# ChainSafe/halo2-verifier

Hardware: AMD Instinct MI355X
Metric: proofs verified/sec (BN254, k=14) (higher is better)
Workload: dtype u32 limbs (254-bit prime-field integers)

## Files before the change

### halo2_verifier_amd/csrc/curve.hip.h

```cpp
#pragma once
#include "bn254.hip.h"

namespace h2v {

static constexpr uint8_t G1_FLAG_IDENTITY = 0x80;
static constexpr uint8_t G1_FLAG_SIGN = 0x40;

struct G1A {
    Fq x, y;
    H2V_HD bool is_identity() const { return x.is_zero() && y.is_zero(); }
    H2V_HD static G1A identity() { G1A p; p.x = Fq::zero(); p.y = Fq::zero(); return p; }
    H2V_HD bool on_curve() const {
        if (is_identity()) return true;
        Fq three = Fq::from_u32(3);
        return y.sqr() == x.sqr() * x + three;
    }
};

struct G1J {
    Fq X, Y, Z;
    H2V_HD static G1J identity() { G1J p; p.X = Fq::zero(); p.Y = Fq::one(); p.Z = Fq::zero(); return p; }
    H2V_HD bool is_identity() const { return Z.is_zero(); }
    H2V_HD static G1J from_affine(const G1A& a) {
        if (a.is_identity()) return identity();
        G1J p; p.X = a.x; p.Y = a.y; p.Z = Fq::one(); return p;
    }
    H2V_HD G1J neg() const { G1J r = *this; r.Y = Y.neg(); return r; }
};

H2V_FN G1J g1_dbl(const G1J& p);
#define H2V_M(a, b) Fq::mul_inl((a), (b))
#define H2V_S(a) (a).sqr_inl()
__host__ __device__ __forceinline__ Fq g1_minus_eight() {
    const Fq k = {{0x1d9096cdu, 0x022be75eu, 0x12c66350u, 0x1e1f47a4u, 0x0b760e9fu, 0x1e7fbbcfu, 0x134a4383u, 0x01be3557u, 0x0022eb3au}};
    return k;
}
__host__ __device__ __forceinline__ G1J g1_dbl_inl(const G1J& p) {
    if (p.is_identity()) return p;
    const Fq A = H2V_S(p.X), B = H2V_S(p.Y), XB = H2V_M(p.X, B), C = H2V_S(B);
    const Fq E = Fq::lazy_add2(A, A), F = H2V_S(E), D = Fq::lazy_dbl(Fq::lazy_dbl(XB));
    int64_t acc[9];
#pragma unroll
    for (int l = 0; l < 9; ++l) acc[l] = (int64_t)F.v[l] + (int64_t)Fq::KP29(9, l) - 2 * (int64_t)D.v[l];
    G1J r;
    r.X = Fq::from_wide(acc);
    r.Y = Fq::dot2_inl(E, Fq::lazy_sub(D, r.X), C, g1_minus_eight());
    r.Z = H2V_M(Fq::lazy_dbl(p.Y), p.Z);
    return r;
}

__host__ __device__ __forceinline__ bool g1_madd_fast(G1J& acc, const G1A& q) {
    if (q.is_identity()) return true;
    if (acc.is_identity()) { acc.X = q.x; acc.Y = q.y; acc.Z = Fq::one(); return true; }
    const Fq Z1Z1 = H2V_S(acc.Z);
    const Fq U2 = H2V_M(q.x, Z1Z1), S2 = H2V_M(H2V_M(q.y, acc.Z), Z1Z1);
    const Fq H = Fq::lazy_sub(U2, acc.X), H2 = Fq::lazy_dbl(H), I = H2V_S(H2);
    if (I.is_zero()) return false;
    const Fq B = Fq::lazy_neg2(acc.Y), rr = Fq::lazy_add2(B, S2);
    const Fq X3 = Fq::dot2_inl(rr, rr, I, Fq::template lazy_lin<8, 1, 2>(H, acc.X));
    const Fq W = Fq::dot2_inl(rr, acc.X, H, B);
    acc.Y = Fq::dot2_inl(I, W, rr, Fq::lazy_neg(X3));
    acc.Z = H2V_M(acc.Z, H2);
    acc.X = X3;
    return true;
}
__host__ __device__ __forceinline__ bool g1_add_fast(G1J& acc, const G1J& q) {
    if (q.is_identity()) return true;
    if (acc.is_identity()) { acc.X = q.X; acc.Y = q.Y; acc.Z = q.Z; return true; }
    const Fq Z1Z1 = H2V_S(acc.Z), Z2Z2 = H2V_S(q.Z);
    const Fq U1 = H2V_M(acc.X, Z2Z2), U2 = H2V_M(q.X, Z1Z1);
    const Fq H = Fq::lazy_sub(U2, U1), H2 = Fq::lazy_dbl(H), I = H2V_S(H2);
    if (I.is_zero()) return false;
    const Fq S1 = H2V_M(H2V_M(acc.Y, q.Z), Z2Z2), S2 = H2V_M(H2V_M(q.Y, acc.Z), Z1Z1);
    const Fq B = Fq::lazy_neg2(S1), rr = Fq::lazy_add2(B, S2);
    const Fq X3 = Fq::dot2_inl(rr, rr, I, Fq::template lazy_lin<8, 1, 2>(H, U1));
    const Fq W = Fq::dot2_inl(rr, U1, H, B);
    acc.Y = Fq::dot2_inl(I, W, rr, Fq::lazy_neg(X3));
    acc.Z = H2V_M(H2V_M(acc.Z, q.Z), H2);
    acc.X = X3;
    return true;
}
__host__ __device__ __forceinline__ G1J g1_add_inl(const G1J& p, const G1J& q) {
    G1J r = p;
    if (g1_add_fast(r, q)) return r;
    const Fq Z1Z1 = H2V_S(p.Z), Z2Z2 = H2V_S(q.Z);
    const Fq S1 = H2V_M(H2V_M(p.Y, q.Z), Z2Z2), S2 = H2V_M(H2V_M(q.Y, p.Z), Z1Z1);
    if (S1 == S2) return g1_dbl(r);
    return G1J::identity();
}

__host__ __device__ __forceinline__ G1J g1_add_affine_inl(const G1J& p, const G1A& q) {
    G1J r = p;
    if (g1_madd_fast(r, q)) return r;
    const Fq Z1Z1 = H2V_S(p.Z);
    const Fq S2 = H2V_M(H2V_M(q.y, p.Z), Z1Z1);
    if (p.Y == S2) return g1_dbl(r);
    return G1J::identity();
}

H2V_FN G1J g1_dbl(const G1J& p) { return g1_dbl_inl(p); }
__host__ __device__ __forceinline__ Fq g1_beta_times(const Fq& x) {
    const Fq beta = {{0x18ccb791u, 0x175b1c3au, 0x0b83d6e2u, 0x0e8ed071u, 0x1282bee2u, 0x04220e84u, 0x1fe4017fu, 0x15084d4au, 0x00169119u}};
    return Fq::mul_inl(x, beta);
}
__host__ __device__ __forceinline__ G1A g1_phi(const G1A& p) { G1A r; r.x = g1_beta_times(p.x); r.y = p.y; return r; }
H2V_FN G1J g1_add(const G1J& p, const G1J& q) { return g1_add_inl(p, q); }
H2V_FN G1J g1_add_affine(const G1J& p, const G1A& q) { return g1_add_affine_inl(p, q); }

H2V_FN G1A g1_to_affine(const G1J& p) {
    if (p.is_identity()) return G1A::identity();
    Fq zi = p.Z.inv(), zi2 = zi.sqr();
    G1A a; a.x = p.X * zi2; a.y = p.Y * zi2 * zi;
    return a;
}

struct FqSqrtSchedule { uint8_t op[400]; int n; };
template <int W> constexpr FqSqrtSchedule fq_sqrt_schedule() {
    constexpr uint32_t e[8] = {0xb61f3f52u, 0x4f082305u, 0x5a1c72a3u, 0x65e05aa4u, 0xa0605617u, 0x6e14116du, 0xb84c680au, 0x0c19139cu};
    FqSqrtSchedule s{};
    s.n = 0;
    int i = 255;
    while (i >= 0 && !((e[i >> 5] >> (i & 31)) & 1)) --i;
    while (i >= 0) {
        if (!((e[i >> 5] >> (i & 31)) & 1)) { s.op[s.n++] = 0; --i; continue; }
        int l = i - (W - 1) < 0 ? 0 : i - (W - 1);
        while (!((e[l >> 5] >> (l & 31)) & 1)) ++l;
        uint32_t v = 0;
        for (int k = i; k >= l; --k) { v = (v << 1) | ((e[k >> 5] >> (k & 31)) & 1); s.op[s.n++] = 0; }
        s.op[s.n++] = (uint8_t)((v + 1) / 2);
        i = l - 1;
    }
    return s;
}
template <int W> __host__ __device__ inline __attribute__((noinline)) Fq fq_sqrt_candidate_w(const Fq& a) {
    constexpr FqSqrtSchedule S = fq_sqrt_schedule<W>();
    constexpr int T = 1 << (W - 1);
    Fq t[T];
    t[0] = a;
    const Fq a2 = a.sqr();
#pragma unroll
    for (int k = 1; k < T; ++k) t[k] = t[k - 1] * a2;
    Fq r = Fq::one();
    bool started = false;
#pragma unroll
    for (int k = 0; k < S.n; ++k) {
        if (S.op[k] == 0) { if (started) r = r.sqr(); }
        else { r = started ? r * t[S.op[k] - 1] : t[S.op[k] - 1]; started = true; }
    }
    return r;
}
H2V_FN Fq fq_sqrt_candidate(const Fq& a) { return fq_sqrt_candidate_w<4>(a); }

struct FqSqrtRuns { uint8_t nsq[160]; uint8_t idx[160]; int n; int first; };
template <int W> constexpr FqSqrtRuns fq_sqrt_runs() {
    constexpr FqSqrtSchedule S = fq_sqrt_schedule<W>();
    FqSqrtRuns r{};
    r.n = 0; r.first = -1;
    int pending = 0;
    for (int k = 0; k < S.n; ++k) {
        if (S.op[k] == 0) { if (r.first >= 0) ++pending; continue; }
        if (r.first < 0) { r.first = S.op[k] - 1; continue; }
        r.nsq[r.n] = (uint8_t)pending; r.idx[r.n] = (uint8_t)(S.op[k] - 1); ++r.n; pending = 0;
    }
    if (pending) { r.nsq[r.n] = (uint8_t)pending; r.idx[r.n] = 255; ++r.n; }
    return r;
}
#if defined(__HIPCC__)
__device__ __constant__ const FqSqrtRuns fq_sqrt_runs_w3 = fq_sqrt_runs<3>();
__device__ __forceinline__ Fq fq_sqrt_candidate_loop_w3(const Fq& a) {
    Fq t0 = a;
    const Fq a2 = a.sqr_inl();
    const Fq t1 = Fq::mul_inl(t0, a2), t2 = Fq::mul_inl(t1, a2), t3 = Fq::mul_inl(t2, a2);
    auto pick = [&](uint32_t i) -> Fq {
        Fq s;
#pragma unroll
        for (int l = 0; l < H2V_LIMBS; ++l) s.v[l] = i == 0 ? t0.v[l] : (i == 1 ? t1.v[l] : (i == 2 ? t2.v[l] : t3.v[l]));
        return s;
    };
    Fq r = pick((uint32_t)fq_sqrt_runs_w3.first);
    const int n = fq_sqrt_runs_w3.n;
#pragma unroll 1
    for (int k = 0; k < n; ++k) {
        const uint32_t nsq = fq_sqrt_runs_w3.nsq[k], idx = fq_sqrt_runs_w3.idx[k];
#pragma unroll 1
        for (uint32_t i = 0; i < nsq; ++i) r = r.sqr_inl();
        if (idx == 0u) r = Fq::mul_inl(r, t0);
        else if (idx == 1u) r = Fq::mul_inl(r, t1);
        else if (idx == 2u) r = Fq::mul_inl(r, t2);
        else if (idx == 3u) r = Fq::mul_inl(r, t3);
    }
    return r;
}
#endif

H2V_FN bool g1_decompress(const uint8_t in[32], G1A& out) {
    uint8_t tmp[32];
    for (int i = 0; i < 32; ++i) tmp[i] = in[i];
    bool is_inf = tmp[31] & G1_FLAG_IDENTITY, sign = tmp[31] & G1_FLAG_SIGN;
    tmp[31] &= 0x3f;
    Fq x;
    if (!Fq::from_bytes(tmp, x)) return false;
    if (is_inf) {
        if (!x.is_zero() || sign) return false;
        out = G1A::identity();
        return true;
    }
    Fq rhs = x.sqr() * x + Fq::from_u32(3);
    Fq y = fq_sqrt_candidate(rhs);
    if (y.sqr() != rhs) return false;
    if (y.is_odd() != sign) y = y.neg();
    out.x = x; out.y = y;
    return true;
}

template <int S> __device__ __forceinline__ Fq quad_bcast(const Fq& v) {
    Fq r;
#pragma unroll
    for (int l = 0; l < H2V_LIMBS; ++l) r.v[l] = (uint32_t)__builtin_amdgcn_mov_dpp((int)v.v[l], S * 0x55, 0xf, 0xf, true);
    return r;
}
__device__ __forceinline__ Fq fq_sel(bool c, const Fq& a, const Fq& b) {
    Fq r;
#pragma unroll
    for (int l = 0; l < H2V_LIMBS; ++l) r.v[l] = c ? a.v[l] : b.v[l];
    return r;
}
__device__ __forceinline__ void g1_dbl_quad(G1J& p, uint32_t r) {
    const Fq Y2 = Fq::lazy_dbl(p.Y);
    const Fq p1 = Fq::mul_inl(fq_sel(r == 0, p.X, fq_sel(r == 1, p.Y, Y2)), fq_sel(r == 0, p.X, fq_sel(r == 1, p.Y, p.Z)));
    const Fq A = quad_bcast<0>(p1), B = quad_bcast<1>(p1), Z3 = quad_bcast<2>(p1);
    const Fq E = Fq::lazy_add2(A, A);
    const Fq p2 = Fq::mul_inl(fq_sel(r == 0, B, fq_sel(r == 1, p.X, E)), fq_sel(r == 2, E, B));
    const Fq C = quad_bcast<0>(p2), XB = quad_bcast<1>(p2), F = quad_bcast<2>(p2);
    const Fq D = Fq::lazy_dbl(Fq::lazy_dbl(XB));
    int64_t acc[9];
#pragma unroll
    for (int l = 0; l < 9; ++l) acc[l] = (int64_t)F.v[l] + (int64_t)Fq::KP29(9, l) - 2 * (int64_t)D.v[l];
    p.X = Fq::from_wide(acc);
    p.Y = Fq::dot2_inl(E, Fq::lazy_sub(D, p.X), C, g1_minus_eight());
    p.Z = Z3;
}
template <class Slot> __device__ __forceinline__ G1J msm_horner_quad(const Slot* __restrict__ src, uint32_t items, uint32_t dbl, uint32_t r) {
    G1J acc = src[items - 1].p;
    for (int w = (int)items - 2; w >= 0; --w) {
        const G1J cur = src[w].p;
#pragma unroll 1
        for (uint32_t i = 0; i < dbl; ++i) g1_dbl_quad(acc, r);
        acc = g1_add_inl(acc, cur);
    }
    return acc;
}

}
```

### halo2_verifier_amd/csrc/internal.h

```cpp
#pragma once
#include <hip/hip_runtime.h>
#include <stdint.h>
#include <string>
#include <vector>
#include "../../include/h2v.h"
#include "curve.hip.h"

namespace h2v {

void set_last_error(const std::string& s);
#define H2V_HIP_CHECK(expr)                                                                     \
    do {                                                                                        \
        hipError_t e_ = (expr);                                                                 \
        if (e_ != hipSuccess) {                                                                 \
            ::h2v::set_last_error(std::string(#expr) + ": " + hipGetErrorString(e_));           \
            return H2V_ERR_DEVICE;                                                              \
        }                                                                                       \
    } while (0)

template <class T> struct DevBuf {
    T* p = nullptr;
    size_t cap = 0;
    DevBuf() {}
    DevBuf(const DevBuf&) = delete;
    DevBuf& operator=(const DevBuf&) = delete;
    DevBuf(DevBuf&& o) noexcept : p(o.p), cap(o.cap) { o.p = nullptr; o.cap = 0; }
    DevBuf& operator=(DevBuf&& o) noexcept { if (this != &o) { reset(); p = o.p; cap = o.cap; o.p = nullptr; o.cap = 0; } return *this; }
    ~DevBuf() { reset(); }
    int alloc(size_t count) {
        reset();
        H2V_HIP_CHECK(hipMalloc(&p, (count ? count : 1) * sizeof(T)));
        cap = count ? count : 1;
        return 0;
    }
    int reserve(size_t count) { return p && count <= cap ? 0 : alloc(count); }
    void reset() { if (p) hipFree(p); p = nullptr; cap = 0; }
};

struct MappedHostBuf {
    uint8_t* p = nullptr;
    void* dev = nullptr;
    size_t cap = 0;
    MappedHostBuf() {}
    MappedHostBuf(const MappedHostBuf&) = delete;
    MappedHostBuf& operator=(const MappedHostBuf&) = delete;
    ~MappedHostBuf() { reset(); }
    int reserve(size_t bytes) {
        if (p && bytes <= cap) return 0;
        reset();
        H2V_HIP_CHECK(hipHostMalloc((void**)&p, bytes ? bytes : 1, hipHostMallocMapped));
        H2V_HIP_CHECK(hipHostGetDevicePointer(&dev, p, 0));
        cap = bytes ? bytes : 1;
        return 0;
    }
    void reset() { if (p) hipHostFree(p); p = nullptr; dev = nullptr; cap = 0; }
};


struct MsmPlan {
    uint32_t n;
    uint32_t c;
    uint32_t windows;
    uint32_t buckets;
};
MsmPlan msm_plan(uint32_t n, bool latency = false);

struct MsmProblem {
    const uint32_t* scalars; const G1A* bases; G1J* out;
    uint32_t sstride, bstride, n;
    uint32_t n1;
    const uint32_t* scalars2; const G1A* bases2;
    const G1A* phi = nullptr; const G1A* phi2 = nullptr;
    uint32_t glv_off = 0;
    uint32_t sub_first = 0, sub_count = 0;
    uint32_t nnz = 0;
    MsmProblem() : scalars(nullptr), bases(nullptr), out(nullptr), sstride(8), bstride(1), n(0), n1(0), scalars2(nullptr), bases2(nullptr) {}
    MsmProblem(const uint32_t* s, const G1A* b, G1J* o, uint32_t ss, uint32_t bs, uint32_t n_) : scalars(s), bases(b), out(o), sstride(ss), bstride(bs), n(n_), n1(n_), scalars2(nullptr), bases2(nullptr) {}
    MsmProblem(const uint32_t* s, const G1A* b, G1J* o, uint32_t ss, uint32_t bs, uint32_t n1_, const uint32_t* s2, const G1A* b2, uint32_t n2)
        : scalars(s), bases(b), out(o), sstride(ss), bstride(bs), n(n1_ + n2), n1(n1_), scalars2(s2), bases2(b2) {}
};
#define MSM_MAX_PROBLEMS 1024
#define MSM_PROBLEM_CHUNK 44
struct MsmProblemChunk { MsmProblem p[MSM_PROBLEM_CHUNK]; };
static_assert(sizeof(MsmProblemChunk) <= 4000, "a chunk of problem descriptors travels as one kernel argument (4 KB limit)");
struct MsmProblems { std::vector<MsmProblem> p; };

struct alignas(128) G1JSlot {
    G1J p;
    uint32_t pad[5];
    __host__ __device__ G1JSlot& operator=(const G1J& v) { p = v; for (int i = 0; i < 5; ++i) pad[i] = 0; return *this; }
    __host__ __device__ operator const G1J&() const { return p; }
};

#define MSM_MAX_PARTS 6
struct MsmSplit {
    uint32_t want_parts = 0;
    uint32_t parts = 0, shift = 0, count = 0;
    const G1JSlot* pts = nullptr;
    const G1JSlot* ready = nullptr;
};

struct AccRecord { uint32_t failed, parts, shift, reserved; G1J left[H2V_ACC_RECORD_PIECES], right[H2V_ACC_RECORD_PIECES]; };
static_assert(sizeof(AccRecord) == H2V_ACC_RECORD_BYTES && H2V_ACC_RECORD_BYTES == 16 + 2 * H2V_ACC_RECORD_PIECES * 108, "accumulator record layout");
static_assert(H2V_ACC_RECORD_PIECES >= MSM_MAX_PARTS, "a record holds every piece a launch can leave");

struct MsmWorkspace {
    uint32_t cap_terms = 0, cap_parents = 0, cap_per_problem = 0;
    uint32_t cap_problems = 0;
    size_t cap_buckets = 0, cap_list = 0;
    DevBuf<uint32_t> counts;
    DevBuf<uint32_t> offsets;
    DevBuf<uint32_t> cursor;
    DevBuf<uint32_t> list;
    DevBuf<G1JSlot> bucket_pts;
    DevBuf<G1JSlot> window_sums;
    DevBuf<G1JSlot> pieces;
    std::vector<MsmProblem> resident;
    int resident_no_split = 0;
    DevBuf<MsmProblem> problems;
    DevBuf<MsmProblem> parents;
    DevBuf<G1JSlot> merged_sums;
    const MsmProblem* final_problems = nullptr;
    DevBuf<uint32_t> block_sums;
    DevBuf<G1JSlot> partial;
    DevBuf<uint32_t> redo;
    DevBuf<uint32_t> glv;
    DevBuf<G1A> phi_pts;
    DevBuf<uint32_t> seg_total;
    DevBuf<uint32_t> seg_start;
    h2v_tuning tune = {};
    bool profile = false, profile_recorded = false;
    hipEvent_t ev_acc[2] = {nullptr, nullptr};
    int reserve(uint32_t max_total_terms, uint32_t max_problems, uint32_t max_terms_per_problem = 0);
    bool covers(uint32_t max_total_terms, uint32_t max_problems, uint32_t max_terms_per_problem = 0) const;
    MsmWorkspace() {}
    MsmWorkspace(const MsmWorkspace&) = delete;
    MsmWorkspace& operator=(const MsmWorkspace&) = delete;
    ~MsmWorkspace() { for (hipEvent_t e : ev_acc) if (e) hipEventDestroy(e); }
};
int msm_enqueue_multi(hipStream_t s, MsmWorkspace& ws, const MsmProblems& pr, MsmSplit* split = nullptr);
int msm_combine_enqueue(hipStream_t s, MsmWorkspace& ws, const MsmSplit& sp, size_t lds_reserve = 0);
#define H2V_AUX_LDS_RESERVE ((size_t)110 * 1024)
int msm_enqueue(hipStream_t s, MsmWorkspace& ws, const uint32_t* d_scalars, const G1A* d_bases, uint32_t n, G1J* d_out);
int accumulator_scale_enqueue(hipStream_t s, const G1J* d_points, const uint32_t* d_scalar_words, void* d_record);
int accumulator_scale_many_enqueue(hipStream_t s, const G1J* d_pairs, const uint32_t* d_slots, const uint32_t* d_scalar_words, uint32_t n, void* d_records);

int bases_from_bytes_enqueue(hipStream_t s, const uint8_t* d_bytes, G1A* d_out, uint32_t* d_flags, uint32_t n);
int scalars_from_bytes_enqueue(hipStream_t s, const uint8_t* d_bytes, uint32_t* d_out, uint32_t* d_flags, uint32_t n);
int copy_words_enqueue(hipStream_t s, const void* d_src, void* d_dst, size_t n_words, size_t lds_reserve = 0);
int point_to_bytes_enqueue(hipStream_t s, const G1J* d_in, uint8_t* d_out_xy64, uint32_t* d_is_identity, uint32_t n, size_t lds_reserve = 0);
int export_records_enqueue(hipStream_t s, const G1J* d_acc, const G1JSlot* d_pieces, uint32_t parts, uint32_t shift, const int* d_status, uint32_t n, uint32_t groups, void* d_out);
int fold_records_enqueue(hipStream_t s, const void* d_recs, uint32_t n_recs, uint32_t groups, uint32_t parts, uint32_t shift, G1J* d_acc, G1JSlot* d_pieces, G1JSlot* d_ready,
                         uint32_t* d_fold_failed);

}
```

### halo2_verifier_amd/csrc/msm.hip

```cpp
#include "../../include/h2v.h"
#include <hip/hip_ext.h>
#include "batch.h"

namespace h2v {

#define MSM_LDS_SORT_MAX_TERMS 16384u
#define MSM_SORT_THREADS 512u
#define MSM_CHUNK_MIN 16u
#define MSM_CHUNK_MAX 64u
#define MSM_ACC_LANES_PER_ROUND 196608u
#define MSM_CHUNK_SMALL 4u
#define MSM_SHORT_LIST 98304u
__host__ __device__ __forceinline__ uint32_t msm_chunk_len(uint32_t E, uint32_t R) {
    if (E <= MSM_SHORT_LIST) return MSM_CHUNK_SMALL;
    if (E <= R * MSM_CHUNK_MIN) return MSM_CHUNK_MIN;
    const uint32_t k = (uint32_t)(((uint64_t)E + (uint64_t)R * MSM_CHUNK_MAX - 1) / ((uint64_t)R * MSM_CHUNK_MAX));
    const uint32_t c = (uint32_t)(((uint64_t)E + (uint64_t)k * R - 1) / ((uint64_t)k * R));
    return c < MSM_CHUNK_MIN ? MSM_CHUNK_MIN : c;
}
static inline uint32_t msm_accumulate_blocks(size_t max_entries, size_t R) {
    size_t lanes;
    if (max_entries <= R * MSM_CHUNK_MIN)
        lanes = std::max<size_t>((max_entries + MSM_CHUNK_MIN - 1) / MSM_CHUNK_MIN, (std::min<size_t>(max_entries, MSM_SHORT_LIST) + MSM_CHUNK_SMALL - 1) / MSM_CHUNK_SMALL);
    else lanes = (max_entries + R * MSM_CHUNK_MAX - 1) / (R * MSM_CHUNK_MAX) * R;
    return (uint32_t)(((lanes + 63) / 64 + 1 + 7) / 8 * 8);
}
#define MSM_CONTROL_WORDS 8u
#define MSM_FIXUP_SERIAL 64u
#define MSM_FIXUP_TEAM 3u
#define MSM_FIXUP_TEAM_BLOCKS 256u
#define MSM_FIXUP_HEAVY_BLOCKS 256u
#define MSM_WIN_THREADS 256

static inline uint32_t msm_window_threads(uint32_t buckets, uint32_t n_workgroups = 0xffffffffu, int forced = 0) {
    if (buckets <= 64) return std::max(1u, buckets);
    if (n_workgroups != 0xffffffffu && (forced == 64 || forced == 128 || forced == 256)) return (uint32_t)forced;
    if (buckets > 2048 || (buckets >= 256 && n_workgroups <= 256)) return 256u;
    return 64u;
}

MsmPlan msm_plan(uint32_t n, bool latency) {
    MsmPlan best{n, 2, 65, 2};
    double best_cost = 1e300;
    for (uint32_t c = 2; c <= 15; ++c) {
        uint32_t w = (130 + c - 1) / c;
        uint32_t b = 1u << (c - 1);
        uint32_t T = msm_window_threads(b), slice = (b + T - 1) / T;
        double lg = 0; for (uint32_t t = T; t > 1; t >>= 1) lg += 1;
        double cost = latency ? 9.0 * w + 9.0 * (2.0 * slice + 1.5 * c + 1.0 + lg) + 5.0 * std::min<double>(32.0, 2.0 * n)
                              : (double)w * (11.0 * 2.0 * n + 16.0 * T * (2.0 * slice + 1.5 * c + 1.0 + lg));
        if (cost < best_cost) { best_cost = cost; best = MsmPlan{n, c, w, b}; }
    }
    return best;
}
static inline bool msm_latency_bound(size_t total_terms) { return total_terms <= 4096; }

static inline uint32_t msm_subproblems(uint32_t n) { return n > MSM_LDS_SORT_MAX_TERMS ? (n + MSM_LDS_SORT_MAX_TERMS - 1) / MSM_LDS_SORT_MAX_TERMS : 1u; }
bool MsmWorkspace::covers(uint32_t max_terms, uint32_t max_problems, uint32_t max_per_problem) const {
    if (!max_per_problem || max_per_problem > max_terms) max_per_problem = max_terms;
    return counts.p && max_terms <= cap_terms && max_problems <= cap_parents && max_per_problem <= cap_per_problem;
}
int MsmWorkspace::reserve(uint32_t max_terms, uint32_t max_problems, uint32_t max_per_problem) {
    if (!max_per_problem || max_per_problem > max_terms) max_per_problem = max_terms;
    if (covers(max_terms, max_problems, max_per_problem)) return 0;
    max_terms = std::max(max_terms, cap_terms); max_problems = std::max(max_problems, cap_parents); max_per_problem = std::max(max_per_problem, cap_per_problem);
    cap_terms = cap_parents = cap_per_problem = 0;
    resident.clear(); final_problems = nullptr; profile_recorded = false;
    const uint32_t subs = msm_subproblems(max_per_problem);
    cap_problems = (uint32_t)std::min<size_t>((size_t)max_problems * subs, MSM_MAX_PROBLEMS);
    if (cap_problems < max_problems) cap_problems = max_problems;
    const uint32_t per_sub = subs > 1 ? MSM_LDS_SORT_MAX_TERMS : max_per_problem;
    const uint32_t form_n[2] = {per_sub, max_per_problem}, form_q[2] = {cap_problems, max_problems};
    size_t mb = 0;
    cap_list = 0;
    for (int f = 0; f < 2; ++f) {
        size_t fb = 0;
        for (int lat = 0; lat < 2; ++lat) {
            for (uint32_t n = 1; n <= form_n[f]; n = n < 16 ? n + 1 : n + n / 8) { MsmPlan p = msm_plan(n, lat != 0); fb = std::max(fb, (size_t)p.windows * p.buckets); }
            MsmPlan p = msm_plan(form_n[f], lat != 0); fb = std::max(fb, (size_t)p.windows * p.buckets);
        }
        mb = std::max(mb, fb * form_q[f]);
        for (uint32_t n = 1;; n = n < 16 ? n + 1 : n + n / 8) {
            if (n > form_n[f]) n = form_n[f];
            size_t terms = n <= MSM_LDS_SORT_MAX_TERMS ? (size_t)n * form_q[f] : std::min<size_t>((size_t)max_terms, (size_t)n * form_q[f]);
            cap_list = std::max(cap_list, terms * 2 * std::max(msm_plan(n, false).windows, msm_plan(n, true).windows));
            if (n == form_n[f]) break;
        }
    }
    cap_buckets = mb;
    const size_t max_chunks = std::max<size_t>(cap_list / MSM_CHUNK_MIN + 1, std::min<size_t>(cap_list, MSM_SHORT_LIST) / MSM_CHUNK_SMALL + 1);
    int rc;
    if ((rc = counts.alloc(mb + MSM_CONTROL_WORDS)) || (rc = offsets.alloc(mb)) ||
        (rc = cursor.alloc(2 * mb)) ||
        (rc = list.alloc(cap_list)) || (rc = bucket_pts.alloc(mb)) || (rc = window_sums.alloc((size_t)128 * cap_problems)) ||
        (rc = merged_sums.alloc((size_t)128 * max_problems)) || (rc = pieces.alloc((size_t)2 * MSM_MAX_PARTS * cap_problems)) ||
        (rc = problems.alloc(cap_problems)) || (rc = parents.alloc(max_problems)) || (rc = block_sums.alloc(mb / 1024 + 2)) ||
        (rc = partial.alloc(max_chunks * 2)) || (rc = redo.alloc(max_chunks)) ||
        (rc = glv.alloc(cap_list / 2 + 1)) ||
        (rc = phi_pts.alloc((size_t)max_terms + 1)) || (rc = seg_total.alloc((size_t)128 * cap_problems + 2)) || (rc = seg_start.alloc((size_t)128 * cap_problems + 2))) {
        cap_problems = 0; cap_buckets = cap_list = 0;
        return rc;
    }
    for (int i = 0; i < 2; ++i) if (!ev_acc[i]) H2V_HIP_CHECK(hipEventCreate(&ev_acc[i]));
    cap_terms = max_terms; cap_parents = max_problems; cap_per_problem = max_per_problem;
    return 0;
}

__device__ __forceinline__ void mul_lo5(uint32_t out[5], const uint32_t* a, int na, const uint32_t* b, int nb) {
    uint64_t acc[5] = {0, 0, 0, 0, 0};
    for (int i = 0; i < na && i < 5; ++i) {
        uint64_t carry = 0;
        for (int j = 0; j < nb && i + j < 5; ++j) {
            uint64_t t = (uint64_t)a[i] * b[j] + (uint32_t)acc[i + j] + carry;
            acc[i + j] = (uint32_t)t; carry = t >> 32;
        }
    }
    for (int i = 0; i < 5; ++i) out[i] = (uint32_t)acc[i];
}
__device__ __forceinline__ void mul_hi256(uint32_t out[5], const uint32_t k[8], const uint32_t g[5]) {
    uint32_t t[13];
    for (int i = 0; i < 13; ++i) t[i] = 0;
    for (int i = 0; i < 8; ++i) {
        uint64_t carry = 0;
        for (int j = 0; j < 5; ++j) {
            uint64_t v = (uint64_t)k[i] * g[j] + t[i + j] + carry;
            t[i + j] = (uint32_t)v; carry = v >> 32;
        }
        t[i + 5] = (uint32_t)carry;
    }
    for (int i = 0; i < 5; ++i) out[i] = t[8 + i];
}
__device__ __forceinline__ void mul_lo8(uint32_t out[8], const uint32_t a[8], const uint32_t* b, int nb) {
    for (int i = 0; i < 8; ++i) out[i] = 0;
    for (int j = 0; j < nb; ++j) {
        uint64_t carry = 0;
        for (int i = 0; i + j < 8; ++i) {
            uint64_t t = (uint64_t)a[i] * b[j] + out[i + j] + carry;
            out[i + j] = (uint32_t)t; carry = t >> 32;
        }
    }
}
__device__ __forceinline__ bool glv_geq_r(const uint32_t v[8]) {
    const uint32_t RW[8] = {0xf0000001u, 0x43e1f593u, 0x79b97091u, 0x2833e848u, 0x8181585du, 0xb85045b6u, 0xe131a029u, 0x30644e72u};
    for (int i = 7; i >= 0; --i) { if (v[i] > RW[i]) return true; if (v[i] < RW[i]) return false; }
    return true;
}
struct GlvHalf { uint32_t mag[5]; bool neg; };
__device__ __forceinline__ void glv_finish(GlvHalf& h, uint32_t t[5]) {
    h.neg = (t[4] >> 31) != 0;
    if (h.neg) { uint64_t c = 1; for (int i = 0; i < 5; ++i) { uint64_t v = (uint64_t)(~t[i]) + c; t[i] = (uint32_t)v; c = v >> 32; } }
    for (int i = 0; i < 5; ++i) h.mag[i] = t[i];
}
__device__ __forceinline__ void glv_decompose(const uint32_t* __restrict__ k, GlvHalf& h1, GlvHalf& h2) {
    const uint32_t A1[5] = {0x7d4f1128u, 0x8211bbebu, 0xeeb859fcu, 0x6f4d8248u, 0u};
    const uint32_t B1N[5] = {0x94d213e3u, 0x89d32568u, 0u, 0u, 0u};
    const uint32_t B2[5] = {0x1221250bu, 0x0be4e154u, 0xeeb859fdu, 0x6f4d8248u, 0u};
    const uint32_t G1[5] = {0x00ff6565u, 0x5398fd03u, 0xa773d2d2u, 0x4ccef014u, 0x2u};
    const uint32_t G2[5] = {0xc7e0b3d7u, 0xd91d232eu, 0x2u, 0u, 0u};
    uint32_t kk[8];
    for (int i = 0; i < 8; ++i) kk[i] = k[i];
    uint32_t c1[5], c2[5], p1[5], p2[5], t1[8], t2[8];
    mul_hi256(c1, kk, G1);
    mul_hi256(c2, kk, G2);
    mul_lo5(p1, c1, 5, A1, 5); mul_lo5(p2, c2, 5, B1N, 5);
    {
        int64_t borrow = 0;
        for (int i = 0; i < 5; ++i) { int64_t v = (int64_t)kk[i] - p1[i] - p2[i] + borrow; t1[i] = (uint32_t)v; borrow = v >> 32; }
    }
    mul_lo5(p1, c1, 5, B1N, 5); mul_lo5(p2, c2, 5, B2, 5);
    {
        int64_t borrow = 0;
        for (int i = 0; i < 5; ++i) { int64_t v = (int64_t)p1[i] - p2[i] + borrow; t2[i] = (uint32_t)v; borrow = v >> 32; }
    }
    {
        const uint32_t s1 = (t1[4] >> 31) ? 0xffffffffu : 0u, s2 = (t2[4] >> 31) ? 0xffffffffu : 0u;
        for (int i = 5; i < 8; ++i) { t1[i] = s1; t2[i] = s2; }
        uint32_t u[8], v[8], w[8];
        mul_lo8(u, t1, B2, 4); mul_lo8(w, t2, B1N, 2);
        { int64_t borrow = 0; for (int i = 0; i < 8; ++i) { int64_t d = (int64_t)u[i] - w[i] + borrow; u[i] = (uint32_t)d; borrow = d >> 32; } }
        mul_lo8(v, t2, A1, 4); mul_lo8(w, t1, B1N, 2);
        { uint64_t carry = 0; for (int i = 0; i < 8; ++i) { uint64_t d = (uint64_t)v[i] + w[i] + carry; v[i] = (uint32_t)d; carry = d >> 32; } }
        const bool e1 = glv_geq_r(u), e2 = glv_geq_r(v);
        int64_t b1 = 0, b2 = 0;
        for (int i = 0; i < 5; ++i) {
            int64_t d = (int64_t)t1[i] - (e1 ? A1[i] : 0u) - (e2 ? B1N[i] : 0u) + b1; t1[i] = (uint32_t)d; b1 = d >> 32;
            d = (int64_t)t2[i] + (e1 ? B1N[i] : 0u) - (e2 ? B2[i] : 0u) + b2; t2[i] = (uint32_t)d; b2 = d >> 32;
        }
    }
    glv_finish(h1, t1);
    glv_finish(h2, t2);
}
__device__ __forceinline__ uint32_t raw_window(const uint32_t m[5], uint32_t w, uint32_t c) {
    uint32_t off = w * c, word = off >> 5, sh = off & 31;
    if (word >= 5) return 0;
    uint32_t v = m[word] >> sh;
    if (sh + c > 32 && word + 1 < 5) v |= m[word + 1] << (32 - sh);
    return v & ((1u << c) - 1);
}
#define ACC_SCALE_TABLE 8u
#define ACC_SCALE_DIGITS 33u
__global__ void __launch_bounds__(64) k_accumulator_scale(const G1J* __restrict__ in, const uint32_t* __restrict__ slots, const uint32_t* __restrict__ scalars,
                                                          AccRecord* __restrict__ out) {
    __shared__ G1J table[4][ACC_SCALE_TABLE];
    __shared__ G1J half_sum[4];
    const uint32_t item = blockIdx.x;
    in += 2 * (size_t)(slots ? slots[item] : item);
    const uint32_t* m_words = scalars + 8 * (size_t)item;
    out += item;
    const uint32_t lane = threadIdx.x, chain = (lane >> 2) & 3u, r = lane & 3u;
    const uint32_t side = chain >> 1, half = chain & 1u;
    const bool writer = lane < 16 && r == 0;
    uint32_t k[8];
    for (int i = 0; i < 8; ++i) k[i] = m_words[i];
    GlvHalf h1, h2;
    glv_decompose(k, h1, h2);
    const bool neg = half ? h2.neg : h1.neg;
    uint32_t mag[5];
    {
        uint64_t c = 0;
        for (int i = 0; i < 5; ++i) { const uint64_t v = (uint64_t)(half ? h2.mag[i] : h1.mag[i]) + (i < 4 ? 0x88888888u : 0x8u) + c; mag[i] = (uint32_t)v; c = v >> 32; }
    }
    G1J p = in[side];
    if (half) p.X = g1_beta_times(p.X);
    if (neg) p.Y = p.Y.neg();
    {
        G1J t = p;
        if (writer) table[chain][0] = t;
        t = g1_dbl(t);
        if (writer) table[chain][1] = t;
#pragma unroll 1
        for (uint32_t j = 2; j < ACC_SCALE_TABLE; ++j) { t = g1_add(t, p); if (writer) table[chain][j] = t; }
    }
    __syncthreads();
    G1J acc = G1J::identity();
#pragma unroll 1
    for (int w = (int)ACC_SCALE_DIGITS - 1; w >= 0; --w) {
        if (w != (int)ACC_SCALE_DIGITS - 1) {
#pragma unroll 1
            for (int i = 0; i < 4; ++i) g1_dbl_quad(acc, r);
        }
        const int d = (int)raw_window(mag, (uint32_t)w, 4) - 8;
        if (d != 0) {
            G1J t = table[chain][(d < 0 ? -d : d) - 1];
            if (d < 0) t.Y = t.Y.neg();
            acc = g1_add_inl(acc, t);
        }
    }
    if (writer) half_sum[chain] = acc;
    __syncthreads();
    if (lane < 2) {
        const G1J a = half_sum[2 * lane], b = half_sum[2 * lane + 1];
        G1J* dst = lane ? out->right : out->left;
        dst[0] = g1_add_inl(a, b);
        for (uint32_t j = 1; j < H2V_ACC_RECORD_PIECES; ++j) dst[j] = G1J::identity();
    }
    if (lane == 0) { out->failed = 0; out->parts = 1; out->shift = 0; out->reserved = 0; }
}
int accumulator_scale_enqueue(hipStream_t s, const G1J* d_points, const uint32_t* d_scalar_words, void* d_record) {
    return accumulator_scale_many_enqueue(s, d_points, nullptr, d_scalar_words, 1, d_record);
}
int accumulator_scale_many_enqueue(hipStream_t s, const G1J* d_pairs, const uint32_t* d_slots, const uint32_t* d_scalar_words, uint32_t n, void* d_records) {
    if (!n) return 0;
    hipLaunchKernelGGL(k_accumulator_scale, dim3(n), dim3(64), 0, s, d_pairs, d_slots, d_scalar_words, (AccRecord*)d_records);
    H2V_HIP_CHECK(hipGetLastError());
    return 0;
}

#define MSM_ENTRY_HALF 0x40000000u
#define MSM_ENTRY_NEG 0x80000000u
#define MSM_ENTRY_TERM 0x3fffffffu

#define MSM_TILE 1024u
#define MSM_TILE_THREADS 256u
#define MSM_LDS_WORDS 16384u

template <bool SCATTER>
__global__ void __launch_bounds__(MSM_TILE_THREADS) msm_count_or_scatter(const MsmProblem* __restrict__ prs, uint32_t n_problems, uint32_t tiles_per_problem, MsmPlan p, uint32_t windows_per_pass, uint32_t* __restrict__ counts,
                                                                         const uint32_t* __restrict__ offsets, uint32_t* __restrict__ cursor, uint32_t* __restrict__ list) {
    extern __shared__ uint32_t hist[];
    const uint32_t tiles = tiles_per_problem, per_xcd = (n_problems + 7) / 8;
    const uint32_t q = (blockIdx.x % 8) * per_xcd + (blockIdx.x / 8) / tiles, tile0 = ((blockIdx.x / 8) % tiles) * MSM_TILE, tid = threadIdx.x;
    if (q >= n_problems) return;
    const MsmProblem pq = prs[q];
    const uint32_t n = pq.n;
    if (tile0 >= n) return;
    const uint32_t nbq = p.windows * p.buckets;
    const uint32_t half_range = 1u << (p.c - 1);
    constexpr uint32_t PER = MSM_TILE / MSM_TILE_THREADS;
    for (uint32_t w0 = 0; w0 < p.windows; w0 += windows_per_pass) {
        const uint32_t w1 = min(p.windows, w0 + windows_per_pass), nwords = (w1 - w0) * p.buckets;
        for (uint32_t i = tid; i < nwords; i += MSM_TILE_THREADS) hist[i] = 0;
        __syncthreads();
        for (int phase = 0; phase < (SCATTER ? 2 : 1); ++phase) {
            for (uint32_t k = 0; k < PER; ++k) {
                const uint32_t t = tile0 + tid + k * MSM_TILE_THREADS;
                if (t >= n) break;
                const uint32_t* s = t < pq.n1 ? pq.scalars + (size_t)pq.sstride * t : pq.scalars2 + (size_t)pq.sstride * (t - pq.n1);
                uint32_t nz = 0;
                for (int i = 0; i < 8; ++i) nz |= s[i];
                if (!nz) continue;
                const uint32_t* bw = reinterpret_cast<const uint32_t*>(t < pq.n1 ? pq.bases + (size_t)pq.bstride * t : pq.bases2 + (size_t)pq.bstride * (t - pq.n1));
                uint32_t any = 0;
                for (int i = 0; i < (int)(sizeof(G1A) / 4); ++i) any |= bw[i];
                if (!any) continue;
                GlvHalf h[2];
                glv_decompose(s, h[0], h[1]);
                for (uint32_t hf = 0; hf < 2; ++hf) {
                    uint32_t carry = 0;
                    for (uint32_t w = 0; w < w1; ++w) {
                        uint32_t raw = raw_window(h[hf].mag, w, p.c) + carry;
                        bool neg_digit = raw > half_range;
                        uint32_t mag = neg_digit ? (1u << p.c) - raw : raw;
                        carry = neg_digit ? 1u : 0u;
                        if (!mag || w < w0) continue;
                        uint32_t local = (w - w0) * p.buckets + mag - 1;
                        if (!SCATTER || phase == 0) atomicAdd(&hist[local], 1u);
                        else {
                            uint32_t b = q * nbq + w * p.buckets + mag - 1;
                            uint32_t pos = atomicAdd(&hist[local], 1u);
                            list[offsets[b] + pos] = t | (hf ? MSM_ENTRY_HALF : 0u) | ((neg_digit != h[hf].neg) ? MSM_ENTRY_NEG : 0u);
                        }
                    }
                }
            }
            __syncthreads();
            if (phase == 0) {
                for (uint32_t i = tid; i < nwords; i += MSM_TILE_THREADS) {
                    uint32_t v = hist[i];
                    if (!v) continue;
                    uint32_t b = q * nbq + w0 * p.buckets + i;
                    if (SCATTER) hist[i] = atomicAdd(&cursor[b], v);
                    else atomicAdd(&counts[b], v);
                }
                __syncthreads();
            }
        }
    }
}

__global__ void __launch_bounds__(256) msm_glv_prep(const MsmProblem* __restrict__ prs, uint32_t n_problems, MsmPlan p, uint32_t* __restrict__ dig, G1A* __restrict__ phi_pts) {
    const uint32_t q = blockIdx.y, t = blockIdx.x * blockDim.x + threadIdx.x;
    if (q >= n_problems) return;
    const MsmProblem pq = prs[q];
    if (t >= pq.n) return;
    uint32_t* out = dig + (size_t)pq.glv_off * p.windows + t;
    const uint32_t* sc = t < pq.n1 ? pq.scalars + (size_t)pq.sstride * t : pq.scalars2 + (size_t)pq.sstride * (t - pq.n1);
    uint32_t nz = 0;
    for (int i = 0; i < 8; ++i) nz |= sc[i];
    if (nz) {
        const uint32_t* bw = reinterpret_cast<const uint32_t*>(t < pq.n1 ? pq.bases + (size_t)pq.bstride * t : pq.bases2 + (size_t)pq.bstride * (t - pq.n1));
        uint32_t any = 0;
        for (int i = 0; i < (int)(sizeof(G1A) / 4); ++i) any |= bw[i];
        nz = any;
        if (any && !(t < pq.n1 ? pq.phi : pq.phi2)) phi_pts[(size_t)pq.glv_off + t] = g1_phi(*reinterpret_cast<const G1A*>(bw));
    }
    if (!nz) { for (uint32_t w = 0; w < p.windows; ++w) out[(size_t)w * pq.n] = 0; return; }
    GlvHalf h[2];
    glv_decompose(sc, h[0], h[1]);
    const uint32_t half_range = 1u << (p.c - 1);
    uint32_t carry[2] = {0, 0};
    for (uint32_t w = 0; w < p.windows; ++w) {
        uint32_t word = 0;
#pragma unroll
        for (uint32_t hf = 0; hf < 2; ++hf) {
            const uint32_t raw = raw_window(h[hf].mag, w, p.c) + carry[hf];
            const bool neg_digit = raw > half_range;
            const uint32_t mag = neg_digit ? (1u << p.c) - raw : raw;
            carry[hf] = neg_digit ? 1u : 0u;
            const uint32_t d16 = mag ? (mag | ((neg_digit != h[hf].neg) ? 0x8000u : 0u)) : 0u;
            word |= d16 << (16 * hf);
        }
        out[(size_t)w * pq.n] = word;
    }
}
__global__ void __launch_bounds__(MSM_SORT_THREADS) msm_sort_lds(const MsmProblem* __restrict__ prs, const uint32_t* __restrict__ dig, MsmPlan p, uint32_t stride,
                                                                 uint32_t* __restrict__ counts, uint32_t* __restrict__ offsets, uint32_t* __restrict__ list,
                                                                 uint32_t* __restrict__ seg_total) {
    extern __shared__ uint32_t sort_lds[];
    uint32_t* hist = sort_lds;
    uint32_t* part = sort_lds + p.buckets;
    unsigned short* rec = reinterpret_cast<unsigned short*>(part + MSM_SORT_THREADS);
    const uint32_t w = blockIdx.x, q = blockIdx.y, tid = threadIdx.x;
    const MsmProblem pq = prs[q];
    const uint32_t n = pq.n, seg = q * p.windows + w;
    const uint32_t* dw = dig + (size_t)pq.glv_off * p.windows + (size_t)w * n;
    for (uint32_t i = tid; i < p.buckets; i += MSM_SORT_THREADS) hist[i] = 0;
    __syncthreads();
    for (int pass = 0; pass < 2; ++pass) {
        for (uint32_t t = tid; t < n; t += MSM_SORT_THREADS) {
            const uint32_t word = dw[t];
#pragma unroll
            for (uint32_t hf = 0; hf < 2; ++hf) {
                const uint32_t d16 = (word >> (16 * hf)) & 0xffffu, mag = d16 & 0x7fffu;
                if (!mag) continue;
                const uint32_t pos = atomicAdd(&hist[mag - 1], 1u);
                if (pass == 1) rec[pos] = (unsigned short)(t | (hf ? 0x4000u : 0u) | (d16 & 0x8000u));
            }
        }
        __syncthreads();
        if (pass == 0) {
            const uint32_t per = (p.buckets + MSM_SORT_THREADS - 1) / MSM_SORT_THREADS, b0 = tid * per;
            uint32_t local = 0;
            for (uint32_t i = 0; i < per; ++i) if (b0 + i < p.buckets) local += hist[b0 + i];
            part[tid] = local;
            __syncthreads();
            for (uint32_t d = 1; d < MSM_SORT_THREADS; d <<= 1) {
                const uint32_t v = tid >= d ? part[tid - d] : 0;
                __syncthreads();
                part[tid] += v;
                __syncthreads();
            }
            uint32_t run = part[tid] - local;
            const size_t bin0 = (size_t)seg * p.buckets;
            for (uint32_t i = 0; i < per; ++i) if (b0 + i < p.buckets) {
                const uint32_t cnt = hist[b0 + i];
                counts[bin0 + b0 + i] = cnt; offsets[bin0 + b0 + i] = run;
                hist[b0 + i] = run;
                run += cnt;
            }
            if (tid == MSM_SORT_THREADS - 1) seg_total[seg] = part[tid];
            __syncthreads();
        }
    }
    const uint32_t total = part[MSM_SORT_THREADS - 1];
    uint32_t* dst = list + (size_t)seg * stride;
    for (uint32_t i = tid; i < total; i += MSM_SORT_THREADS) {
        const uint32_t r = rec[i];
        dst[i] = (r & 0x3fffu) | ((r & 0x4000u) ? MSM_ENTRY_HALF : 0u) | ((r & 0x8000u) ? MSM_ENTRY_NEG : 0u);
    }
}
__global__ void __launch_bounds__(1024) msm_seg_scan(const uint32_t* __restrict__ seg_total, uint32_t nseg, uint32_t* __restrict__ seg_start, uint32_t* __restrict__ control) {
    __shared__ uint32_t part[1024];
    __shared__ uint32_t carry;
    const uint32_t t = threadIdx.x;
    if (t == 0) carry = 0;
    __syncthreads();
    for (uint32_t base = 0; base < nseg; base += 1024) {
        const uint32_t i = base + t, c = i < nseg ? seg_total[i] : 0;
        part[t] = c;
        __syncthreads();
        for (uint32_t d = 1; d < 1024; d <<= 1) {
            const uint32_t v = t >= d ? part[t - d] : 0;
            __syncthreads();
            part[t] += v;
            __syncthreads();
        }
        if (i < nseg) seg_start[i] = carry + part[t] - c;
        __syncthreads();
        if (t == 1023) carry += part[1023];
        __syncthreads();
    }
    if (t == 0) { seg_start[nseg] = carry; control[0] = 0; control[1] = carry; control[2] = 0; control[3] = 0; control[4] = 0; }
}

__device__ __forceinline__ G1A msm_entry_load(const MsmProblem& q, uint32_t e, const G1A* __restrict__ phi_pts) {
    const uint32_t t = e & MSM_ENTRY_TERM;
    const bool first = t < q.n1;
    const size_t off = (size_t)(first ? t : t - q.n1) * q.bstride;
    const G1A* b = (first ? q.bases : q.bases2) + off;
    if (phi_pts && (e & MSM_ENTRY_HALF)) {
        const G1A* ph = first ? q.phi : q.phi2;
        b = ph ? ph + off : phi_pts + ((size_t)q.glv_off + t);
    }
    return *b;
}
__device__ __forceinline__ G1A msm_entry_apply(G1A b, uint32_t e, bool have_phi) {
    if (!have_phi && (e & MSM_ENTRY_HALF)) b.x = g1_beta_times(b.x);
    if ((e & MSM_ENTRY_NEG) && !b.y.is_zero()) b.y = Fq::lazy_neg(b.y);
    return b;
}
__device__ __forceinline__ G1A msm_entry_base(const MsmProblem& q, uint32_t e) { return msm_entry_apply(msm_entry_load(q, e, nullptr), e, false); }

__global__ void __launch_bounds__(1024) msm_block_sums(const uint32_t* __restrict__ counts, uint32_t* __restrict__ block_sums, uint32_t nb) {
    __shared__ uint32_t part[1024];
    const uint32_t t = threadIdx.x, i = blockIdx.x * 1024 + t;
    part[t] = i < nb ? counts[i] : 0;
    __syncthreads();
    for (uint32_t d = 512; d > 0; d >>= 1) { if (t < d) part[t] += part[t + d]; __syncthreads(); }
    if (t == 0) block_sums[blockIdx.x] = part[0];
}
__global__ void __launch_bounds__(1024) msm_scan_sums(uint32_t* __restrict__ block_sums, uint32_t nblk, uint32_t* __restrict__ total) {
    __shared__ uint32_t part[1024];
    __shared__ uint32_t carry;
    const uint32_t t = threadIdx.x;
    if (t == 0) carry = 0;
    __syncthreads();
    for (uint32_t base = 0; base < nblk; base += 1024) {
        const uint32_t i = base + t;
        const uint32_t c = i < nblk ? block_sums[i] : 0;
        part[t] = c;
        __syncthreads();
        for (uint32_t d = 1; d < 1024; d <<= 1) {
            uint32_t v = t >= d ? part[t - d] : 0;
            __syncthreads();
            part[t] += v;
            __syncthreads();
        }
        if (i < nblk) block_sums[i] = carry + part[t] - c;
        __syncthreads();
        if (t == 1023) carry += part[1023];
        __syncthreads();
    }
    if (t == 0) *total = carry;
}
__global__ void __launch_bounds__(1024) msm_offsets(const uint32_t* __restrict__ counts, const uint32_t* __restrict__ block_sums, uint32_t* __restrict__ offsets,
                                                    uint32_t* __restrict__ cursor, uint32_t nb) {
    __shared__ uint32_t part[1024];
    const uint32_t t = threadIdx.x, i = blockIdx.x * 1024 + t;
    const uint32_t c = i < nb ? counts[i] : 0;
    part[t] = c;
    __syncthreads();
    for (uint32_t d = 1; d < 1024; d <<= 1) {
        uint32_t v = t >= d ? part[t - d] : 0;
        __syncthreads();
        part[t] += v;
        __syncthreads();
    }
    if (i < nb) { offsets[i] = block_sums[blockIdx.x] + part[t] - c; cursor[i] = 0; }
}

struct MsmSeg { const uint32_t* seg_start; uint32_t nseg, bps, stride, lanes_round; };
__device__ __forceinline__ uint32_t msm_bin_start(const MsmSeg& g, const uint32_t* __restrict__ offsets, uint32_t b) { return g.seg_start[b / g.bps] + offsets[b]; }
__device__ __forceinline__ uint32_t msm_bin_of(const MsmSeg& g, const uint32_t* __restrict__ offsets, uint32_t pos) {
    uint32_t lo = 0, hi = g.nseg;
    while (hi - lo > 1) { uint32_t mid = (lo + hi) >> 1; if (g.seg_start[mid] <= pos) lo = mid; else hi = mid; }
    const uint32_t base = lo * g.bps, local = pos - g.seg_start[lo];
    lo = 0; hi = g.bps;
    while (hi - lo > 1) { uint32_t mid = (lo + hi) >> 1; if (offsets[base + mid] <= local) lo = mid; else hi = mid; }
    return base + lo;
}
__device__ __forceinline__ G1JSlot* msm_piece_dst(G1JSlot* __restrict__ bucket_pts, G1JSlot* __restrict__ partial, uint32_t lane, uint32_t b, uint32_t bin_lo, uint32_t bin_hi,
                                              uint32_t chunk_lo, uint32_t chunk_hi, bool first) {
    if (bin_lo >= chunk_lo && bin_hi <= chunk_hi) return bucket_pts + b;
    return partial + 2 * (size_t)lane + (first ? 0 : 1);
}
__device__ __noinline__ void msm_chunk_slow(const MsmProblem* __restrict__ prs, uint32_t nbq, const uint32_t* __restrict__ counts, const uint32_t* __restrict__ offsets,
                                            const uint32_t* __restrict__ list, G1JSlot* __restrict__ bucket_pts, G1JSlot* __restrict__ partial, uint32_t nb, uint32_t lane, uint32_t E, MsmSeg g) {
    const uint32_t CH = msm_chunk_len(E, g.lanes_round);
    const uint32_t chunk_lo = lane * CH, chunk_hi = min(chunk_lo + CH, E);
    uint32_t b = msm_bin_of(g, offsets, chunk_lo);
    uint32_t bin_lo = msm_bin_start(g, offsets, b), bin_hi = bin_lo + counts[b];
    MsmProblem q = prs[b / nbq];
    G1J acc = G1J::identity();
    bool first = true;
    for (uint32_t pos = chunk_lo; pos < chunk_hi;) {
        const uint32_t sg = b / g.bps;
        acc = g1_add_affine(acc, msm_entry_base(q, list[(size_t)sg * g.stride + (pos - g.seg_start[sg])]));
        ++pos;
        if (pos == bin_hi || pos == chunk_hi) {
            *msm_piece_dst(bucket_pts, partial, lane, b, bin_lo, bin_hi, chunk_lo, chunk_hi, first) = acc;
            acc = G1J::identity(); first = false;
            if (pos == bin_hi && pos < chunk_hi) {
                { uint32_t tries = 0; do { ++b; } while (counts[b] == 0 && ++tries < 2); if (counts[b] == 0) b = msm_bin_of(g, offsets, pos); }
                bin_lo = bin_hi; bin_hi = bin_lo + counts[b];
                q = prs[b / nbq];
            }
        }
    }
}
__device__ __forceinline__ void msm_chunk_tail(uint32_t b, uint32_t bin_lo, uint32_t bin_hi, uint32_t chunk_lo, uint32_t chunk_hi, uint32_t CH, uint32_t lane, uint32_t nb,
                                               uint32_t* __restrict__ control, uint32_t* __restrict__ lists) {
    if (bin_hi > chunk_hi && bin_lo >= chunk_lo) {
        const uint32_t span = (bin_hi - 1) / CH - lane;
        if (span >= MSM_FIXUP_SERIAL) lists[nb - 1 - atomicAdd(&control[0], 1u)] = b;
        else if (span >= MSM_FIXUP_TEAM) lists[nb + atomicAdd(&control[3], 1u)] = b;
        else lists[atomicAdd(&control[2], 1u)] = b;
    }
}
__device__ __forceinline__ void msm_accumulate_chunk(const MsmProblem* __restrict__ prs, uint32_t nbq, const uint32_t* __restrict__ counts, const uint32_t* __restrict__ offsets,
                                                     const uint32_t* __restrict__ list, G1JSlot* __restrict__ bucket_pts, G1JSlot* __restrict__ partial, uint32_t nb, const MsmSeg& g,
                                                     uint32_t* __restrict__ control, uint32_t* __restrict__ lists, const G1A* __restrict__ phi_pts, uint32_t* __restrict__ redo, uint32_t E, uint32_t CH,
                                                     uint32_t lane) {
    const uint32_t chunk_lo = lane * CH;
    if (chunk_lo >= E) return;
    const uint32_t chunk_hi = min(chunk_lo + CH, E);
    uint32_t b = msm_bin_of(g, offsets, chunk_lo);
    uint32_t sg = b / g.bps, seg_lo = g.seg_start[sg];
    uint32_t bin_lo = seg_lo + offsets[b], bin_hi = bin_lo + counts[b];
    uint32_t qi = b / nbq;
    MsmProblem q = prs[qi];
    G1J acc = G1J::identity();
    bool first = true, ok = true;
    uint32_t e_next = list[(size_t)sg * g.stride + (chunk_lo - seg_lo)];
    G1A raw_next = msm_entry_load(q, e_next, phi_pts);
    for (uint32_t pos = chunk_lo; pos < chunk_hi && ok;) {
        const uint32_t e = e_next;
        const G1A raw = raw_next;
        ++pos;
        const bool flush = pos == bin_hi || pos == chunk_hi;
        uint32_t b_next = b, lo_next = bin_lo, hi_next = bin_hi, qn = qi;
        MsmProblem q_next = q;
        if (pos == bin_hi && pos < chunk_hi) {
            uint32_t tries = 0;
            do { ++b_next; } while (counts[b_next] == 0 && ++tries < 2);
            if (counts[b_next] == 0) b_next = msm_bin_of(g, offsets, pos);
            lo_next = bin_hi; hi_next = lo_next + counts[b_next];
            const uint32_t sn = b_next / g.bps;
            if (sn != sg) { sg = sn; seg_lo = g.seg_start[sn]; }
            qn = b_next / nbq;
            if (qn != qi) q_next = prs[qn];
        }
        const uint32_t pos_n = min(pos, chunk_hi - 1);
        e_next = list[(size_t)sg * g.stride + (pos_n - seg_lo)]; raw_next = msm_entry_load(q_next, e_next, phi_pts);
        ok = g1_madd_fast(acc, msm_entry_apply(raw, e, phi_pts != nullptr));
        if (flush) {
            if (ok) *msm_piece_dst(bucket_pts, partial, lane, b, bin_lo, bin_hi, chunk_lo, chunk_hi, first) = acc;
            acc = G1J::identity(); first = false;
        }
        b = b_next; bin_lo = lo_next; bin_hi = hi_next; qi = qn; q = q_next;
    }
    if (!ok) { redo[atomicAdd(&control[4], 1u)] = lane; return; }
    msm_chunk_tail(b, bin_lo, bin_hi, chunk_lo, chunk_hi, CH, lane, nb, control, lists);
}
__global__ void __launch_bounds__(64) __attribute__((amdgpu_waves_per_eu(3, 3))) msm_accumulate(const MsmProblem* __restrict__ prs, uint32_t nbq, const uint32_t* __restrict__ counts, const uint32_t* __restrict__ offsets,
                                                     const uint32_t* __restrict__ list, G1JSlot* __restrict__ bucket_pts, G1JSlot* __restrict__ partial, uint32_t nb, MsmSeg g,
                                                     uint32_t* __restrict__ control, uint32_t* __restrict__ lists, const G1A* __restrict__ phi_pts, uint32_t* __restrict__ redo) {
    const uint32_t E = counts[nb + 1];
    const uint32_t CH = msm_chunk_len(E, g.lanes_round);
    const uint32_t blocks = ((E + CH - 1) / CH + 63) / 64, per_xcd = (blocks + 7) / 8;
    for (uint32_t j = blockIdx.x / 8; j < per_xcd; j += gridDim.x / 8)
        msm_accumulate_chunk(prs, nbq, counts, offsets, list, bucket_pts, partial, nb, g, control, lists, phi_pts, redo, E, CH, ((blockIdx.x % 8) * per_xcd + j) * 64 + threadIdx.x);
}
__global__ void __launch_bounds__(64) msm_accumulate_redo(const MsmProblem* __restrict__ prs, uint32_t nbq, const uint32_t* __restrict__ counts, const uint32_t* __restrict__ offsets,
                                                          const uint32_t* __restrict__ list, G1JSlot* __restrict__ bucket_pts, G1JSlot* __restrict__ partial, uint32_t nb, MsmSeg g,
                                                          uint32_t* __restrict__ control, uint32_t* __restrict__ lists, const uint32_t* __restrict__ redo) {
    const uint32_t n_redo = control[4], E = counts[nb + 1], CH = msm_chunk_len(E, g.lanes_round);
    for (uint32_t i = blockIdx.x * blockDim.x + threadIdx.x; i < n_redo; i += gridDim.x * blockDim.x) {
        const uint32_t lane = redo[i], chunk_lo = lane * CH, chunk_hi = min(chunk_lo + CH, E);
        msm_chunk_slow(prs, nbq, counts, offsets, list, bucket_pts, partial, nb, lane, E, g);
        const uint32_t b = msm_bin_of(g, offsets, chunk_hi - 1), bin_lo = msm_bin_start(g, offsets, b), bin_hi = bin_lo + counts[b];
        msm_chunk_tail(b, bin_lo, bin_hi, chunk_lo, chunk_hi, CH, lane, nb, control, lists);
    }
}

__device__ __forceinline__ const G1JSlot* msm_piece_src(const G1JSlot* __restrict__ partial, uint32_t i, uint32_t i0, uint32_t off, uint32_t CH) {
    return partial + 2 * (size_t)i + ((i == i0 && off > i0 * CH) ? 1 : 0);
}
__device__ __noinline__ void msm_fixup_slow(const G1JSlot* __restrict__ partial, uint32_t i0, uint32_t i1, uint32_t off, uint32_t CH, G1JSlot* __restrict__ out) {
    G1J acc = msm_piece_src(partial, i0, i0, off, CH)->p;
    for (uint32_t i = i0 + 1; i <= i1; ++i) acc = g1_add(acc, msm_piece_src(partial, i, i0, off, CH)->p);
    *out = acc;
}
__device__ __noinline__ void g1_add_to(G1J* dst, const G1J* a, const G1J* b);
__device__ __noinline__ void msm_fixup_team(const uint32_t* __restrict__ counts, const uint32_t* __restrict__ offsets, const G1JSlot* __restrict__ partial,
                                            const uint32_t* __restrict__ lists, G1JSlot* __restrict__ bucket_pts, uint32_t nb, const MsmSeg& g, G1J* team_acc) {
    const uint32_t n_team = counts[nb + 3], r = threadIdx.x & 7u;
    const uint32_t CH = msm_chunk_len(counts[nb + 1], g.lanes_round);
    for (uint32_t m0 = blockIdx.x * 8; m0 < n_team; m0 += MSM_FIXUP_TEAM_BLOCKS * 8) {
        const uint32_t m = m0 + (threadIdx.x >> 3);
        const bool live = m < n_team;
        const uint32_t b = live ? lists[nb + m] : 0;
        const uint32_t cnt = live ? counts[b] : 0, off = live ? msm_bin_start(g, offsets, b) : 0;
        const uint32_t i0 = off / CH, i1 = cnt ? (off + cnt - 1) / CH : i0;
        G1J* mine = team_acc + threadIdx.x;
        *mine = G1J::identity();
        if (live) for (uint32_t i = i0 + r; i <= i1; i += 8) g1_add_to(mine, mine, &msm_piece_src(partial, i, i0, off, CH)->p);
        for (uint32_t d = 4; d > 0; d >>= 1)
            g1_add_to(mine, mine, team_acc + min(threadIdx.x + d, 63u));
        if (live && r == 0) bucket_pts[b] = *mine;
    }
}
__device__ __noinline__ void msm_fixup_heavy(const uint32_t* __restrict__ counts, const uint32_t* __restrict__ offsets, const G1JSlot* __restrict__ partial,
                                             const uint32_t* __restrict__ lists, G1JSlot* __restrict__ bucket_pts, uint32_t nb, const MsmSeg& g, uint32_t first_block) {
    const uint32_t n_heavy = counts[nb], t = threadIdx.x;
    const uint32_t CH = msm_chunk_len(counts[nb + 1], g.lanes_round);
    for (uint32_t h = blockIdx.x - first_block; h < n_heavy; h += MSM_FIXUP_HEAVY_BLOCKS) {
        const uint32_t b = lists[nb - 1 - h];
        const uint32_t cnt = counts[b], off = msm_bin_start(g, offsets, b);
        const uint32_t i0 = off / CH, i1 = (off + cnt - 1) / CH;
        G1J acc = G1J::identity();
        for (uint32_t i = i0 + t; i <= i1; i += 64) acc = g1_add(acc, msm_piece_src(partial, i, i0, off, CH)->p);
        for (uint32_t d = 32; d > 0; d >>= 1) {
            G1J other;
            uint32_t* dst = reinterpret_cast<uint32_t*>(&other);
            const uint32_t* src = reinterpret_cast<const uint32_t*>(&acc);
#pragma unroll
            for (uint32_t k = 0; k < sizeof(G1J) / 4; ++k) dst[k] = (uint32_t)__shfl_down((int)src[k], d, 64);
            acc = g1_add(acc, other);
        }
        if (t == 0) bucket_pts[b] = acc;
    }
}
__global__ void __launch_bounds__(64) msm_fixup(const uint32_t* __restrict__ counts, const uint32_t* __restrict__ offsets, const G1JSlot* __restrict__ partial,
                                                const uint32_t* __restrict__ lists, G1JSlot* __restrict__ bucket_pts, uint32_t nb, MsmSeg g) {
    __shared__ G1J team_acc[64];
    if (blockIdx.x < MSM_FIXUP_TEAM_BLOCKS) { msm_fixup_team(counts, offsets, partial, lists, bucket_pts, nb, g, team_acc); return; }
    if (blockIdx.x < MSM_FIXUP_TEAM_BLOCKS + MSM_FIXUP_HEAVY_BLOCKS) { msm_fixup_heavy(counts, offsets, partial, lists, bucket_pts, nb, g, MSM_FIXUP_TEAM_BLOCKS); return; }
    const uint32_t k = (blockIdx.x - MSM_FIXUP_TEAM_BLOCKS - MSM_FIXUP_HEAVY_BLOCKS) * blockDim.x + threadIdx.x;
    if (k >= counts[nb + 2]) return;
    const uint32_t b = lists[k];
    const uint32_t cnt = counts[b], off = msm_bin_start(g, offsets, b);
    const uint32_t CH = msm_chunk_len(counts[nb + 1], g.lanes_round);
    const uint32_t i0 = off / CH, i1 = (off + cnt - 1) / CH;
    G1J acc = msm_piece_src(partial, i0, i0, off, CH)->p;
    bool ok = true;
    for (uint32_t i = i0 + 1; i <= i1 && ok; ++i) ok = g1_add_fast(acc, msm_piece_src(partial, i, i0, off, CH)->p);
    if (!ok) { msm_fixup_slow(partial, i0, i1, off, CH, bucket_pts + b); return; }
    bucket_pts[b] = acc;
}
#define MSM_WIN_SLOTS 5
__device__ __noinline__ void g1_add_to(G1J* dst, const G1J* a, const G1J* b) { const G1J x = *a, y = *b; *dst = g1_add_inl(x, y); }
__device__ __noinline__ void g1_dbl_to(G1J* dst, const G1J* a) { const G1J x = *a; *dst = g1_dbl_inl(x); }

__global__ void __launch_bounds__(MSM_WIN_THREADS) msm_window(const G1JSlot* __restrict__ bucket_pts, const uint32_t* __restrict__ counts, G1JSlot* __restrict__ window_sums, MsmPlan p,
                                                              uint32_t n_windows, uint32_t wpw, uint32_t slots) {
    __builtin_amdgcn_s_setprio(3);
    extern __shared__ G1J win_lds[];
    const uint32_t T = blockDim.x / wpw, sub = threadIdx.x / T, t = threadIdx.x % T;
    const uint32_t widx = blockIdx.x * wpw + sub;
    const bool live = widx < n_windows;
    G1J* mine = win_lds + (size_t)sub * slots * T;
    G1J* run = mine + t;
    G1J* sum = mine + T + t;
    G1J* scaled = mine + 2 * T + t;
    G1J* red = mine + 2 * T;
    const uint32_t slice = (p.buckets + T - 1) / T;
    const uint32_t lo = live ? min(p.buckets, t * slice) : 0, hi = live ? min(p.buckets, lo + slice) : 0;
    *run = G1J::identity(); *sum = G1J::identity();
    const G1JSlot* bp = bucket_pts + (size_t)widx * p.buckets;
    const uint32_t* cn = counts + (size_t)widx * p.buckets;
    for (uint32_t b = hi; b > lo; --b) {
        if (cn[b - 1]) g1_add_to(run, run, &bp[b - 1].p);
        g1_add_to(sum, sum, run);
    }
    if ((slice & (slice - 1)) == 0 && T > 1 && slots >= MSM_WIN_SLOTS) {
        G1J* run2 = mine + 3 * T + t;
        G1J* run3 = mine + 4 * T + t;
        if (lo < hi && t > 0) {
            g1_dbl_to(run2, run);
            g1_add_to(run3, run2, run);
            *scaled = G1J::identity();
            const int nd = (32 - (int)__clz((int)(T - 1)) + 1) / 2;
            for (int d = nd - 1; d >= 0; --d) {
                if (d < nd - 1) { g1_dbl_to(scaled, scaled); g1_dbl_to(scaled, scaled); }
                const uint32_t dig = (t >> (2 * d)) & 3u;
                if (dig) g1_add_to(scaled, scaled, dig == 1 ? run : (dig == 2 ? run2 : run3));
            }
            for (uint32_t w = slice; w > 1; w >>= 1) g1_dbl_to(scaled, scaled);
            g1_add_to(sum, sum, scaled);
        }
    } else if (lo < hi && lo > 0) {
        const int top = 31 - (int)__clz((int)lo);
        *scaled = G1J::identity();
        for (int i = top; i >= 0; --i) {
            if (i < top) g1_dbl_to(scaled, scaled);
            if ((lo >> i) & 1) g1_add_to(scaled, scaled, run);
        }
        g1_add_to(sum, sum, scaled);
    }
    if (blockDim.x <= 64) {
        for (uint32_t d = 32; d > 0; d >>= 1) {
            const G1J mine_sum = *sum;
            G1J other;
            uint32_t* dst = reinterpret_cast<uint32_t*>(&other);
            const uint32_t* src = reinterpret_cast<const uint32_t*>(&mine_sum);
#pragma unroll
            for (uint32_t k = 0; k < sizeof(G1J) / 4; ++k) dst[k] = (uint32_t)__shfl_down((int)src[k], d, 64);
            if (t + d >= T) other = G1J::identity();
            *scaled = other;
            g1_add_to(sum, sum, scaled);
        }
        if (t == 0 && live) window_sums[widx] = *sum;
        return;
    }
    const uint32_t W = T < 64u ? T : 64u;
    for (uint32_t d = W / 2; d > 0; d >>= 1) {
        const G1J mine_sum = *sum;
        G1J other;
        uint32_t* dst = reinterpret_cast<uint32_t*>(&other);
        const uint32_t* src = reinterpret_cast<const uint32_t*>(&mine_sum);
#pragma unroll
        for (uint32_t k = 0; k < sizeof(G1J) / 4; ++k) dst[k] = (uint32_t)__shfl_down((int)src[k], d, 64);
        if ((t & (W - 1)) + d >= W) other = G1J::identity();
        *scaled = other;
        g1_add_to(sum, sum, scaled);
    }
    __syncthreads();
    if ((t & (W - 1)) == 0) red[t >> 6] = *sum;
    __syncthreads();
    if (t == 0) {
        for (uint32_t wv = 1; wv < (T >> 6); ++wv) g1_add_to(&red[0], &red[0], &red[wv]);
        if (live) window_sums[widx] = red[0];
    }
}

__global__ void __launch_bounds__(64) msm_final(const G1JSlot* __restrict__ window_sums, const MsmProblem* __restrict__ prs, uint32_t count, MsmPlan p) {
    __builtin_amdgcn_s_setprio(3);
    const uint32_t t = blockIdx.x * blockDim.x + threadIdx.x, q = t >> 2, r = t & 3u;
    if (q >= count) return;
    G1J acc = G1J::identity();
    if (prs[q].n) acc = msm_horner_quad(window_sums + (size_t)q * p.windows, p.windows, p.c, r);
    if (r == 0) *prs[q].out = acc;
}
__global__ void __launch_bounds__(64) msm_final_parts(const G1JSlot* __restrict__ window_sums, const MsmProblem* __restrict__ prs, uint32_t count, MsmPlan p,
                                                      uint32_t parts, uint32_t wpp, G1JSlot* __restrict__ out, G1JSlot* __restrict__ ready) {
    __builtin_amdgcn_s_setprio(3);
    const uint32_t t = blockIdx.x * blockDim.x + threadIdx.x, quad = t >> 2, r = t & 3u;
    if (quad >= count * parts) return;
    const uint32_t q = quad / parts, j = quad % parts, lo = j * wpp, hi = min(p.windows, lo + wpp);
    G1J acc = G1J::identity();
    if (prs[q].n && lo < hi) acc = msm_horner_quad(window_sums + (size_t)q * p.windows + lo, hi - lo, p.c, r);
    if (r == 0) out[quad] = acc;
    if (r == 0) { ready[quad].p.X = Fq::mul_inl(acc.X, acc.Z); ready[quad].p.Y = acc.Y; }
    if (r == 1) ready[quad].p.Z = Fq::mul_inl(acc.Z.sqr_inl(), acc.Z);
}
__global__ void __launch_bounds__(64) msm_combine_parts(const G1JSlot* __restrict__ pieces, const MsmProblem* __restrict__ prs, uint32_t count, uint32_t parts, uint32_t shift) {
    const uint32_t t = blockIdx.x * blockDim.x + threadIdx.x, q = t >> 2, r = t & 3u;
    if (q >= count) return;
    const G1J acc = msm_horner_quad(pieces + (size_t)q * parts, parts, shift, r);
    if (r == 0) *prs[q].out = acc;
}

__global__ void __launch_bounds__(64) msm_merge_windows(const G1JSlot* __restrict__ sub_sums, const MsmProblem* __restrict__ parents, uint32_t n_parents, uint32_t windows,
                                                        G1JSlot* __restrict__ merged) {
    const uint32_t team = (blockIdx.x * blockDim.x + threadIdx.x) >> 3, r = threadIdx.x & 7u;
    const bool live = team < n_parents * windows;
    const uint32_t q = live ? team / windows : 0, w = live ? team % windows : 0;
    const uint32_t first = parents[q].sub_first, cnt = live ? parents[q].sub_count : 0;
    G1J acc = G1J::identity();
    for (uint32_t k = r; k < cnt; k += 8) acc = g1_add(acc, sub_sums[(size_t)(first + k) * windows + w].p);
    for (uint32_t d = 4; d > 0; d >>= 1) {
        G1J other;
        uint32_t* dst = reinterpret_cast<uint32_t*>(&other);
        const uint32_t* src = reinterpret_cast<const uint32_t*>(&acc);
#pragma unroll
        for (uint32_t k = 0; k < sizeof(G1J) / 4; ++k) dst[k] = (uint32_t)__shfl_down((int)src[k], d, 8);
        acc = g1_add(acc, other);
    }
    if (live && r == 0) merged[(size_t)q * windows + w] = acc;
}

__global__ void msm_set_problems(MsmProblemChunk ch, uint32_t count, MsmProblem* __restrict__ dst) {
    uint32_t i = threadIdx.x;
    if (i < count) dst[i] = ch.p[i];
}

static MsmProblem msm_problem_slice(const MsmProblem& q, uint32_t first, uint32_t len) {
    MsmProblem r = q;
    r.out = nullptr; r.n = len; r.nnz = 0; r.sub_first = 0; r.sub_count = 0;
    if (first < q.n1) {
        r.scalars = q.scalars + (size_t)q.sstride * first; r.bases = q.bases + (size_t)q.bstride * first;
        if (q.phi) r.phi = q.phi + (size_t)q.bstride * first;
        r.n1 = std::min(q.n1 - first, len);
    } else {
        r.scalars = q.scalars2 + (size_t)q.sstride * (first - q.n1); r.bases = q.bases2 + (size_t)q.bstride * (first - q.n1);
        r.phi = q.phi2 ? q.phi2 + (size_t)q.bstride * (first - q.n1) : nullptr;
        r.n1 = len; r.scalars2 = nullptr; r.bases2 = nullptr; r.phi2 = nullptr;
    }
    return r;
}
static void msm_upload_problems(hipStream_t s, const std::vector<MsmProblem>& v, bool assign_glv, MsmProblem* dst) {
    uint32_t glv_next = 0;
    const uint32_t count = (uint32_t)v.size();
    for (uint32_t q0 = 0; q0 < count; q0 += MSM_PROBLEM_CHUNK) {
        MsmProblemChunk ch;
        uint32_t k = std::min<uint32_t>(MSM_PROBLEM_CHUNK, count - q0);
        for (uint32_t i = 0; i < k; ++i) { ch.p[i] = v[q0 + i]; if (assign_glv) { ch.p[i].glv_off = glv_next; glv_next += v[q0 + i].n; } }
        hipLaunchKernelGGL(msm_set_problems, dim3(1), dim3(64), 0, s, ch, k, dst + q0);
    }
}

struct MsmLaunchShape { std::vector<MsmProblem> launch_p, parents_p; bool cut = false; uint32_t nmax = 0; size_t total = 0, total_nz = 0; };
static int msm_shape(const MsmWorkspace& ws, const MsmProblems& pr, MsmLaunchShape& L) {
    const uint32_t n_callers = (uint32_t)pr.p.size();
    if (n_callers > MSM_MAX_PROBLEMS || n_callers > std::max(ws.cap_problems, ws.cap_parents)) { set_last_error("msm_enqueue_multi: too many problems"); return H2V_ERR_BAD_ARGUMENT; }
    for (uint32_t q = 0; q < n_callers; ++q) { L.nmax = std::max(L.nmax, pr.p[q].n); L.total += pr.p[q].n; L.total_nz += pr.p[q].nnz ? std::min(pr.p[q].nnz, pr.p[q].n) : pr.p[q].n; }
    if (L.nmax > MSM_LDS_SORT_MAX_TERMS && !ws.tune.msm_no_term_split) {
        size_t subs = 0;
        for (uint32_t q = 0; q < n_callers; ++q) subs += msm_subproblems(pr.p[q].n);
        L.cut = subs <= ws.cap_problems && subs <= MSM_MAX_PROBLEMS && n_callers <= ws.cap_parents;
    }
    if (L.cut) {
        for (uint32_t q = 0; q < n_callers; ++q) {
            const MsmProblem& c = pr.p[q];
            const uint32_t k = msm_subproblems(c.n), per = (c.n + k - 1) / k;
            MsmProblem parent = c;
            parent.sub_first = (uint32_t)L.launch_p.size(); parent.sub_count = k;
            for (uint32_t i = 0; i < k; ++i) { const uint32_t first = std::min(c.n, i * per); L.launch_p.push_back(msm_problem_slice(c, first, std::min(per, c.n - first))); }
            L.parents_p.push_back(parent);
        }
        L.nmax = 0;
        for (const MsmProblem& q : L.launch_p) L.nmax = std::max(L.nmax, q.n);
    } else {
        if (n_callers > ws.cap_problems) { set_last_error("msm_enqueue_multi: too many problems"); return H2V_ERR_BAD_ARGUMENT; }
        L.launch_p = pr.p;
    }
    return 0;
}
static bool msm_same_problems(const std::vector<MsmProblem>& a, const std::vector<MsmProblem>& b) {
    if (a.size() != b.size()) return false;
    for (size_t i = 0; i < a.size(); ++i) {
        const MsmProblem &x = a[i], &y = b[i];
        if (x.scalars != y.scalars || x.bases != y.bases || x.out != y.out || x.sstride != y.sstride || x.bstride != y.bstride || x.n != y.n || x.n1 != y.n1 ||
            x.scalars2 != y.scalars2 || x.bases2 != y.bases2 || x.phi != y.phi || x.phi2 != y.phi2 || x.nnz != y.nnz) return false;
    }
    return true;
}
int msm_enqueue_multi(hipStream_t s, MsmWorkspace& ws, const MsmProblems& pr, MsmSplit* split) {
    if (split) { split->parts = 0; split->shift = 0; split->count = 0; split->pts = nullptr; split->ready = nullptr; }
    const uint32_t n_callers = (uint32_t)pr.p.size();
    if (n_callers == 0) return 0;
    MsmLaunchShape L;
    { int rc = msm_shape(ws, pr, L); if (rc) return rc; }
    const bool cut = L.cut;
    uint32_t nmax = L.nmax; const size_t total = L.total, total_nz = L.total_nz;
    const std::vector<MsmProblem>& launch_p = L.launch_p;
    const bool uploaded = !ws.resident.empty() && ws.resident_no_split == ws.tune.msm_no_term_split && msm_same_problems(ws.resident, pr.p);
    if (!uploaded) {
        if (cut) msm_upload_problems(s, L.parents_p, false, ws.parents.p);
        msm_upload_problems(s, launch_p, true, ws.problems.p);
        ws.resident = pr.p; ws.resident_no_split = ws.tune.msm_no_term_split;
    }
    const uint32_t count = (uint32_t)launch_p.size();
    ws.final_problems = cut ? ws.parents.p : ws.problems.p;
    if (nmax == 0) {
        hipLaunchKernelGGL(msm_final, dim3((4 * count + 63) / 64), dim3(64), 0, s, ws.window_sums.p, ws.problems.p, count, MsmPlan{0, 2, 0, 3});
        H2V_HIP_CHECK(hipGetLastError());
        return 0;
    }
    if (nmax > MSM_ENTRY_TERM) { set_last_error("msm_enqueue_multi: more than 2^30 terms in one problem"); return H2V_ERR_BAD_ARGUMENT; }
    if (total > ws.cap_terms) { set_last_error("msm_enqueue_multi: terms exceed workspace capacity"); return H2V_ERR_BAD_ARGUMENT; }
    MsmPlan p = msm_plan(nmax, msm_latency_bound(total));
    uint32_t nbq = p.windows * p.buckets, nb = nbq * count;
    if (nb > ws.cap_buckets || total * 2 * p.windows > ws.cap_list) { set_last_error("msm_enqueue_multi: workspace too small"); return H2V_ERR_BAD_ARGUMENT; }
    const uint32_t stride = 2 * nmax;
    const size_t sort_lds = ((size_t)p.buckets + MSM_SORT_THREADS) * 4 + (size_t)stride * 2;
    const bool lds_sort = nmax <= MSM_LDS_SORT_MAX_TERMS && sort_lds <= 150 * 1024 && (size_t)count * p.windows * stride <= ws.cap_list &&
                          (size_t)count * p.windows <= (size_t)128 * ws.cap_problems && !ws.tune.msm_global_sort;
    MsmSeg g;
    if (lds_sort) {
        hipLaunchKernelGGL(msm_glv_prep, dim3((nmax + 255) / 256, count), dim3(256), 0, s, ws.problems.p, count, p, ws.glv.p, ws.phi_pts.p);
        if (sort_lds > 64 * 1024) H2V_HIP_CHECK(hipFuncSetAttribute((const void*)msm_sort_lds, hipFuncAttributeMaxDynamicSharedMemorySize, (int)sort_lds));
        hipLaunchKernelGGL(msm_sort_lds, dim3(p.windows, count), dim3(MSM_SORT_THREADS), sort_lds, s, ws.problems.p, ws.glv.p, p, stride, ws.counts.p, ws.offsets.p, ws.list.p, ws.seg_total.p);
        hipLaunchKernelGGL(msm_seg_scan, dim3(1), dim3(1024), 0, s, ws.seg_total.p, p.windows * count, ws.seg_start.p, ws.counts.p + nb);
        g = MsmSeg{ws.seg_start.p, p.windows * count, p.buckets, stride, MSM_ACC_LANES_PER_ROUND};
    } else {
    H2V_HIP_CHECK(hipMemsetAsync(ws.counts.p, 0, ((size_t)nb + MSM_CONTROL_WORDS) * 4, s));
    H2V_HIP_CHECK(hipMemsetAsync(ws.seg_start.p, 0, 4, s));
    const uint32_t tiles = (nmax + MSM_TILE - 1) / MSM_TILE;
    dim3 gt(8 * ((count + 7) / 8) * tiles);
    const uint32_t wpp = std::max<uint32_t>(1u, std::min<uint32_t>(p.windows, MSM_LDS_WORDS / p.buckets));
    const size_t lds = (size_t)wpp * p.buckets * 4;
    hipLaunchKernelGGL(msm_count_or_scatter<false>, gt, dim3(MSM_TILE_THREADS), lds, s, ws.problems.p, count, tiles, p, wpp, ws.counts.p, ws.offsets.p, ws.cursor.p, ws.list.p);
    const uint32_t nblk = (nb + 1023) / 1024;
    hipLaunchKernelGGL(msm_block_sums, dim3(nblk), dim3(1024), 0, s, ws.counts.p, ws.block_sums.p, nb);
    hipLaunchKernelGGL(msm_scan_sums, dim3(1), dim3(1024), 0, s, ws.block_sums.p, nblk, ws.counts.p + nb + 1);
    hipLaunchKernelGGL(msm_offsets, dim3(nblk), dim3(1024), 0, s, ws.counts.p, ws.block_sums.p, ws.offsets.p, ws.cursor.p, nb);
    hipLaunchKernelGGL(msm_count_or_scatter<true>, gt, dim3(MSM_TILE_THREADS), lds, s, ws.problems.p, count, tiles, p, wpp, ws.counts.p, ws.offsets.p, ws.cursor.p, ws.list.p);
    g = MsmSeg{ws.seg_start.p, 1, nb, 0, MSM_ACC_LANES_PER_ROUND};
    }
    const uint32_t acc_blocks = msm_accumulate_blocks(total_nz * 2 * p.windows, MSM_ACC_LANES_PER_ROUND);
    {
        const G1A* phi_tab = lds_sort ? (const G1A*)ws.phi_pts.p : (const G1A*)nullptr;
        if (ws.profile) {
            hipExtLaunchKernelGGL(msm_accumulate, dim3(acc_blocks), dim3(64), 0, s, ws.ev_acc[0], ws.ev_acc[1], 0, ws.problems.p, nbq, ws.counts.p, ws.offsets.p, ws.list.p, ws.bucket_pts.p, ws.partial.p, nb, g, ws.counts.p + nb, ws.cursor.p, phi_tab, ws.redo.p);
            ws.profile_recorded = true;
        } else hipLaunchKernelGGL(msm_accumulate, dim3(acc_blocks), dim3(64), 0, s, ws.problems.p, nbq, ws.counts.p, ws.offsets.p, ws.list.p, ws.bucket_pts.p, ws.partial.p, nb, g, ws.counts.p + nb, ws.cursor.p, phi_tab, ws.redo.p);
    }
    hipLaunchKernelGGL(msm_accumulate_redo, dim3(256), dim3(64), 0, s, ws.problems.p, nbq, ws.counts.p, ws.offsets.p, ws.list.p, ws.bucket_pts.p, ws.partial.p, nb, g, ws.counts.p + nb, ws.cursor.p, ws.redo.p);
    hipLaunchKernelGGL(msm_fixup, dim3((nb + 63) / 64 + MSM_FIXUP_TEAM_BLOCKS + MSM_FIXUP_HEAVY_BLOCKS), dim3(64), 0, s, ws.counts.p, ws.offsets.p, ws.partial.p, ws.cursor.p, ws.bucket_pts.p, nb, g);
    {
        const uint32_t nw = p.windows * count;
        uint32_t T = msm_window_threads(p.buckets, nw, ws.tune.msm_window_threads), wpw = 1;
        if (T == 64 && p.buckets >= 256 && nw > 256 && nw <= 512 && !ws.tune.msm_window_threads) { T = 128; wpw = 2; }
        const uint32_t wpw_forced = (uint32_t)ws.tune.msm_window_wpw;
        if ((wpw_forced == 1 || wpw_forced == 2 || wpw_forced == 4) && T * wpw_forced <= MSM_WIN_THREADS) wpw = wpw_forced;
        const uint32_t slots = ((T * wpw <= 64 && nw > 1024) || ws.tune.msm_window_slots == 3) ? 3u : (uint32_t)MSM_WIN_SLOTS;
        const size_t win_lds = (size_t)slots * T * wpw * sizeof(G1J);
        if (win_lds > 64 * 1024) H2V_HIP_CHECK(hipFuncSetAttribute((const void*)msm_window, hipFuncAttributeMaxDynamicSharedMemorySize, (int)win_lds));
        hipLaunchKernelGGL(msm_window, dim3((nw + wpw - 1) / wpw), dim3(T * wpw), win_lds, s, ws.bucket_pts.p, ws.counts.p, ws.window_sums.p, p, nw, wpw, slots);
    }
    const G1JSlot* sums = ws.window_sums.p;
    if (cut) {
        hipLaunchKernelGGL(msm_merge_windows, dim3((8 * n_callers * p.windows + 63) / 64), dim3(64), 0, s, ws.window_sums.p, ws.parents.p, n_callers, p.windows, ws.merged_sums.p);
        sums = ws.merged_sums.p;
    }
    if (split && split->want_parts > 1 && p.windows > 1) {
        const uint32_t want = std::min<uint32_t>(split->want_parts, MSM_MAX_PARTS);
        const uint32_t wpp = (p.windows + want - 1) / want, parts = (p.windows + wpp - 1) / wpp;
        hipLaunchKernelGGL(msm_final_parts, dim3((4 * n_callers * parts + 63) / 64), dim3(64), 0, s, sums, ws.final_problems, n_callers, p, parts, wpp, ws.pieces.p, ws.pieces.p + (size_t)MSM_MAX_PARTS * ws.cap_problems);
        split->parts = parts; split->shift = p.c * wpp; split->count = n_callers; split->pts = ws.pieces.p; split->ready = ws.pieces.p + (size_t)MSM_MAX_PARTS * ws.cap_problems;
    } else {
        hipLaunchKernelGGL(msm_final, dim3((4 * n_callers + 63) / 64), dim3(64), 0, s, sums, ws.final_problems, n_callers, p);
    }
    H2V_HIP_CHECK(hipGetLastError());
    return 0;
}
int msm_combine_enqueue(hipStream_t s, MsmWorkspace& ws, const MsmSplit& sp, size_t lds_reserve) {
    if (!sp.parts) return 0;
    if (lds_reserve > 64 * 1024) H2V_HIP_CHECK(hipFuncSetAttribute((const void*)msm_combine_parts, hipFuncAttributeMaxDynamicSharedMemorySize, (int)lds_reserve));
    hipLaunchKernelGGL(msm_combine_parts, dim3((4 * sp.count + 63) / 64), dim3(64), lds_reserve, s, sp.pts, ws.final_problems, sp.count, sp.parts, sp.shift);
    H2V_HIP_CHECK(hipGetLastError());
    return 0;
}

int msm_enqueue(hipStream_t s, MsmWorkspace& ws, const uint32_t* d_scalars, const G1A* d_bases, uint32_t n, G1J* d_out) {
    MsmProblems pr;
    pr.p.push_back(MsmProblem(d_scalars, d_bases, d_out, 8, 1, n));
    return msm_enqueue_multi(s, ws, pr);
}

}
```

Baseline: 11.75 million.

## Use narrower variable-width windows for small MSM problems in batched launches

Adds a narrow-window path for small problems in a batched MSM. Each small problem's 128-bit GLV half-scalars are re-digitized into sub-windows whose width is chosen by a chain-length cost model. Several sub-windows are packed into one bucket segment, and each sub-window is reduced by a few lanes inside the same window kernel. The final Horner step then doubles by per-sub-window widths. The goal is to shorten the serial bucket-reduction chain, which is long with wide c-bit windows when each problem has only a handful of terms. The cost is more sub-windows, more digit rows to sort and extra class-table uploads, plus considerable added complexity in the sort, window and final kernels.

```diff
diff --git a/halo2_verifier_amd/csrc/curve.hip.h b/halo2_verifier_amd/csrc/curve.hip.h
--- a/halo2_verifier_amd/csrc/curve.hip.h
+++ b/halo2_verifier_amd/csrc/curve.hip.h
@@ -250,5 +250,16 @@
     }
     return acc;
 }
-
-}
+template <class Slot, class Sub> __device__ __forceinline__ G1J msm_horner_quad_widths(const Slot* __restrict__ src, const Sub* __restrict__ sub, uint32_t items, uint32_t r) {
+    G1J acc = src[items - 1].p;
+    for (int w = (int)items - 2; w >= 0; --w) {
+        const G1J cur = src[w].p;
+        const uint32_t dbl = sub[w].width;
+#pragma unroll 1
+        for (uint32_t i = 0; i < dbl; ++i) g1_dbl_quad(acc, r);
+        acc = g1_add_inl(acc, cur);
+    }
+    return acc;
+}
+
+}
diff --git a/halo2_verifier_amd/csrc/internal.h b/halo2_verifier_amd/csrc/internal.h
--- a/halo2_verifier_amd/csrc/internal.h
+++ b/halo2_verifier_amd/csrc/internal.h
@@ -57,11 +57,15 @@
 };
 
 
+struct MsmNarrowClass;
+struct MsmNarrowProblem;
 struct MsmPlan {
     uint32_t n;
     uint32_t c;
     uint32_t windows;
     uint32_t buckets;
+    const MsmNarrowClass* narrow = nullptr;
+    const MsmNarrowProblem* narrow_q = nullptr;
 };
 MsmPlan msm_plan(uint32_t n, bool latency = false);
 
@@ -93,6 +97,31 @@
 };
 
 #define MSM_MAX_PARTS 6
+
+#define MSM_NARROW_CLASSES 4
+#define MSM_NARROW_SUBS 48
+#define MSM_NARROW_LANES 8u
+#define MSM_NARROW_MIN_C 8u
+#define MSM_NARROW_BITS 128u
+struct MsmNarrowSub { uint16_t off, width; uint32_t bin; };
+struct MsmNarrowClass {
+    uint32_t n_max;
+    uint32_t subs;
+    uint32_t c;
+    uint32_t lanes;
+    uint32_t piece_first[MSM_MAX_PARTS + 1];
+    MsmNarrowSub sub[MSM_NARROW_SUBS];
+};
+struct MsmNarrowProblem {
+    uint32_t cls;
+    uint32_t dig_off;
+    uint32_t sum_off;
+};
+#define MSM_NARROW_PROBLEM_CHUNK 256
+struct MsmNarrowProblemChunk { MsmNarrowProblem q[MSM_NARROW_PROBLEM_CHUNK]; };
+struct MsmNarrowTable { MsmNarrowClass cls[MSM_NARROW_CLASSES]; };
+static_assert(sizeof(MsmNarrowTable) <= 4000, "the class table travels as one kernel argument");
+bool msm_narrow_class(const MsmPlan& p, uint32_t wpp, uint32_t nmax, uint32_t n, MsmNarrowClass& out);
 struct MsmSplit {
     uint32_t want_parts = 0;
     uint32_t parts = 0, shift = 0, count = 0;
@@ -128,6 +157,10 @@
     DevBuf<G1A> phi_pts;
     DevBuf<uint32_t> seg_total;
     DevBuf<uint32_t> seg_start;
+    DevBuf<MsmNarrowClass> narrow_tab;
+    DevBuf<MsmNarrowProblem> narrow_q;
+    MsmNarrowTable narrow_host = {};
+    bool resident_narrow = false;
     h2v_tuning tune = {};
     bool profile = false, profile_recorded = false;
     hipEvent_t ev_acc[2] = {nullptr, nullptr};
diff --git a/halo2_verifier_amd/csrc/msm.hip b/halo2_verifier_amd/csrc/msm.hip
--- a/halo2_verifier_amd/csrc/msm.hip
+++ b/halo2_verifier_amd/csrc/msm.hip
@@ -1,5 +1,6 @@
 #include "../../include/h2v.h"
 #include <hip/hip_ext.h>
+#include <cstring>
 #include "batch.h"
 
 namespace h2v {
@@ -55,6 +56,61 @@
 }
 static inline bool msm_latency_bound(size_t total_terms) { return total_terms <= 4096; }
 
+static inline double msm_wide_chain(uint32_t buckets, uint32_t T, uint32_t c) {
+    double lg = 0; for (uint32_t t = T; t > 1; t >>= 1) lg += 1;
+    return 2.0 * ((buckets + T - 1) / T) + 1.5 * c + 1.0 + lg;
+}
+static inline double msm_narrow_chain(uint32_t buckets, uint32_t lanes) {
+    const uint32_t T = std::min(lanes, buckets), slice = buckets / T;
+    double lg = 0, ls = 0;
+    for (uint32_t t = T; t > 1; t >>= 1) lg += 1;
+    for (uint32_t t = slice; t > 1; t >>= 1) ls += 1;
+    return 2.0 * slice + 1.5 * lg + 0.5 * ls + 1.0 + lg;
+}
+static bool msm_narrow_layout(const MsmPlan& p, uint32_t wpp, uint32_t nmax, uint32_t n, uint32_t cn, MsmNarrowClass& out) {
+    const uint32_t parts = (p.windows + wpp - 1) / wpp;
+    if (parts > MSM_MAX_PARTS) return false;
+    memset(&out, 0, sizeof(out));
+    out.n_max = n; out.lanes = MSM_NARROW_LANES;
+    uint32_t bin = 0, seg = 0, seg_entries = 0;
+    for (uint32_t j = 0; j < parts; ++j) {
+        out.piece_first[j] = out.subs;
+        const uint32_t lo = std::min<uint32_t>(MSM_NARROW_BITS, j * wpp * p.c), hi = std::min<uint32_t>(MSM_NARROW_BITS, (j + 1) * wpp * p.c), span = hi - lo;
+        const uint32_t k = (span + cn - 1) / cn;
+        for (uint32_t i = 0, off = lo; i < k; ++i) {
+            const uint32_t width = span / k + (i < span % k ? 1u : 0u), nbk = 1u << (width - 1);
+            if (out.subs == MSM_NARROW_SUBS) return false;
+            if (bin / p.buckets != seg) { seg = bin / p.buckets; seg_entries = 0; }
+            if (bin % p.buckets + nbk > p.buckets || seg_entries + 2 * n > 2 * nmax) { bin = (seg + 1) * p.buckets; seg += 1; seg_entries = 0; }
+            out.sub[out.subs++] = MsmNarrowSub{(uint16_t)off, (uint16_t)width, bin};
+            out.c = std::max(out.c, width);
+            bin += nbk; seg_entries += 2 * n; off += width;
+        }
+    }
+    for (uint32_t j = parts; j <= MSM_MAX_PARTS; ++j) out.piece_first[j] = out.subs;
+    return out.subs > 0 && bin <= p.windows * p.buckets;
+}
+#define MSM_NARROW_GAIN 1.5
+bool msm_narrow_class(const MsmPlan& p, uint32_t wpp, uint32_t nmax, uint32_t n, MsmNarrowClass& out) {
+    if (p.c < MSM_NARROW_MIN_C || n == 0 || n > nmax || wpp == 0) return false;
+    const uint32_t T = msm_window_threads(p.buckets);
+    const double wide_chain = msm_wide_chain(p.buckets, T, p.c);
+    const double launch_cost = (double)p.windows * (11.0 * 2.0 * n + 16.0 * T * wide_chain);
+    double best_cost = 1e300;
+    MsmNarrowClass cand;
+    for (uint32_t cn = 2; cn < p.c; ++cn) {
+        if (msm_narrow_chain(1u << (cn - 1), MSM_NARROW_LANES) > wide_chain) break;
+        if (!msm_narrow_layout(p, wpp, nmax, n, cn, cand)) continue;
+        double cost = 0;
+        for (uint32_t s = 0; s < cand.subs; ++s) {
+            const uint32_t b = 1u << (cand.sub[s].width - 1);
+            cost += 11.0 * 2.0 * n + 16.0 * MSM_NARROW_LANES * msm_narrow_chain(b, MSM_NARROW_LANES);
+        }
+        if (cost < best_cost) { best_cost = cost; out = cand; }
+    }
+    return best_cost * MSM_NARROW_GAIN <= launch_cost;
+}
+
 static inline uint32_t msm_subproblems(uint32_t n) { return n > MSM_LDS_SORT_MAX_TERMS ? (n + MSM_LDS_SORT_MAX_TERMS - 1) / MSM_LDS_SORT_MAX_TERMS : 1u; }
 bool MsmWorkspace::covers(uint32_t max_terms, uint32_t max_problems, uint32_t max_per_problem) const {
     if (!max_per_problem || max_per_problem > max_terms) max_per_problem = max_terms;
@@ -65,7 +121,7 @@
     if (covers(max_terms, max_problems, max_per_problem)) return 0;
     max_terms = std::max(max_terms, cap_terms); max_problems = std::max(max_problems, cap_parents); max_per_problem = std::max(max_per_problem, cap_per_problem);
     cap_terms = cap_parents = cap_per_problem = 0;
-    resident.clear(); final_problems = nullptr; profile_recorded = false;
+    resident.clear(); resident_narrow = false; final_problems = nullptr; profile_recorded = false;
     const uint32_t subs = msm_subproblems(max_per_problem);
     cap_problems = (uint32_t)std::min<size_t>((size_t)max_problems * subs, MSM_MAX_PROBLEMS);
     if (cap_problems < max_problems) cap_problems = max_problems;
@@ -97,7 +153,8 @@
         (rc = problems.alloc(cap_problems)) || (rc = parents.alloc(max_problems)) || (rc = block_sums.alloc(mb / 1024 + 2)) ||
         (rc = partial.alloc(max_chunks * 2)) || (rc = redo.alloc(max_chunks)) ||
         (rc = glv.alloc(cap_list / 2 + 1)) ||
-        (rc = phi_pts.alloc((size_t)max_terms + 1)) || (rc = seg_total.alloc((size_t)128 * cap_problems + 2)) || (rc = seg_start.alloc((size_t)128 * cap_problems + 2))) {
+        (rc = phi_pts.alloc((size_t)max_terms + 1)) || (rc = seg_total.alloc((size_t)128 * cap_problems + 2)) || (rc = seg_start.alloc((size_t)128 * cap_problems + 2)) ||
+        (rc = narrow_tab.alloc(MSM_NARROW_CLASSES)) || (rc = narrow_q.alloc(cap_problems))) {
         cap_problems = 0; cap_buckets = cap_list = 0;
         return rc;
     }
@@ -190,13 +247,14 @@
     glv_finish(h1, t1);
     glv_finish(h2, t2);
 }
-__device__ __forceinline__ uint32_t raw_window(const uint32_t m[5], uint32_t w, uint32_t c) {
-    uint32_t off = w * c, word = off >> 5, sh = off & 31;
+__device__ __forceinline__ uint32_t raw_bits(const uint32_t m[5], uint32_t off, uint32_t c) {
+    uint32_t word = off >> 5, sh = off & 31;
     if (word >= 5) return 0;
     uint32_t v = m[word] >> sh;
     if (sh + c > 32 && word + 1 < 5) v |= m[word + 1] << (32 - sh);
     return v & ((1u << c) - 1);
 }
+__device__ __forceinline__ uint32_t raw_window(const uint32_t m[5], uint32_t w, uint32_t c) { return raw_bits(m, w * c, c); }
 #define ACC_SCALE_TABLE 8u
 #define ACC_SCALE_DIGITS 33u
 __global__ void __launch_bounds__(64) k_accumulator_scale(const G1J* __restrict__ in, const uint32_t* __restrict__ slots, const uint32_t* __restrict__ scalars,
@@ -343,7 +401,10 @@
     if (q >= n_problems) return;
     const MsmProblem pq = prs[q];
     if (t >= pq.n) return;
-    uint32_t* out = dig + (size_t)pq.glv_off * p.windows + t;
+    const MsmNarrowProblem nq = p.narrow ? p.narrow_q[q] : MsmNarrowProblem{0, 0, 0};
+    uint32_t* out = dig + (p.narrow ? (size_t)nq.dig_off : (size_t)pq.glv_off * p.windows) + t;
+    const MsmNarrowClass* nc = nq.cls ? p.narrow + (nq.cls - 1) : nullptr;
+    const uint32_t rows = nc ? nc->subs : p.windows;
     const uint32_t* sc = t < pq.n1 ? pq.scalars + (size_t)pq.sstride * t : pq.scalars2 + (size_t)pq.sstride * (t - pq.n1);
     uint32_t nz = 0;
     for (int i = 0; i < 8; ++i) nz |= sc[i];
@@ -354,11 +415,28 @@
         nz = any;
         if (any && !(t < pq.n1 ? pq.phi : pq.phi2)) phi_pts[(size_t)pq.glv_off + t] = g1_phi(*reinterpret_cast<const G1A*>(bw));
     }
-    if (!nz) { for (uint32_t w = 0; w < p.windows; ++w) out[(size_t)w * pq.n] = 0; return; }
+    if (!nz) { for (uint32_t w = 0; w < rows; ++w) out[(size_t)w * pq.n] = 0; return; }
     GlvHalf h[2];
     glv_decompose(sc, h[0], h[1]);
+    uint32_t carry[2] = {0, 0};
+    if (nc) {
+        for (uint32_t w = 0; w < rows; ++w) {
+            const MsmNarrowSub sb = nc->sub[w];
+            uint32_t word = 0;
+#pragma unroll
+            for (uint32_t hf = 0; hf < 2; ++hf) {
+                const uint32_t raw = raw_bits(h[hf].mag, sb.off, sb.width) + carry[hf];
+                const bool neg_digit = raw > (1u << (sb.width - 1));
+                const uint32_t mag = neg_digit ? (1u << sb.width) - raw : raw;
+                carry[hf] = neg_digit ? 1u : 0u;
+                const uint32_t d16 = mag ? (mag | ((neg_digit != h[hf].neg) ? 0x8000u : 0u)) : 0u;
+                word |= d16 << (16 * hf);
+            }
+            out[(size_t)w * pq.n] = word;
+        }
+        return;
+    }
     const uint32_t half_range = 1u << (p.c - 1);
-    uint32_t carry[2] = {0, 0};
     for (uint32_t w = 0; w < p.windows; ++w) {
         uint32_t word = 0;
 #pragma unroll
@@ -383,19 +461,32 @@
     const uint32_t w = blockIdx.x, q = blockIdx.y, tid = threadIdx.x;
     const MsmProblem pq = prs[q];
     const uint32_t n = pq.n, seg = q * p.windows + w;
-    const uint32_t* dw = dig + (size_t)pq.glv_off * p.windows + (size_t)w * n;
+    const MsmNarrowProblem nq = p.narrow ? p.narrow_q[q] : MsmNarrowProblem{0, 0, 0};
+    const MsmNarrowClass* nc = nq.cls ? p.narrow + (nq.cls - 1) : nullptr;
+    uint32_t row_lo = w, row_hi = w + 1;
+    if (nc) {
+        row_lo = 0;
+        while (row_lo < nc->subs && nc->sub[row_lo].bin / p.buckets < w) ++row_lo;
+        row_hi = row_lo;
+        while (row_hi < nc->subs && nc->sub[row_hi].bin / p.buckets == w) ++row_hi;
+    }
+    const uint32_t* dq = dig + (p.narrow ? (size_t)nq.dig_off : (size_t)pq.glv_off * p.windows);
     for (uint32_t i = tid; i < p.buckets; i += MSM_SORT_THREADS) hist[i] = 0;
     __syncthreads();
     for (int pass = 0; pass < 2; ++pass) {
+        for (uint32_t row = row_lo; row < row_hi; ++row) {
+        const uint32_t* dw = dq + (size_t)row * n;
+        const uint32_t bin0 = nc ? nc->sub[row].bin - w * p.buckets : 0u;
         for (uint32_t t = tid; t < n; t += MSM_SORT_THREADS) {
             const uint32_t word = dw[t];
 #pragma unroll
             for (uint32_t hf = 0; hf < 2; ++hf) {
                 const uint32_t d16 = (word >> (16 * hf)) & 0xffffu, mag = d16 & 0x7fffu;
                 if (!mag) continue;
-                const uint32_t pos = atomicAdd(&hist[mag - 1], 1u);
+                const uint32_t pos = atomicAdd(&hist[bin0 + mag - 1], 1u);
                 if (pass == 1) rec[pos] = (unsigned short)(t | (hf ? 0x4000u : 0u) | (d16 & 0x8000u));
             }
+        }
         }
         __syncthreads();
         if (pass == 0) {
@@ -702,13 +793,66 @@
 __device__ __noinline__ void g1_add_to(G1J* dst, const G1J* a, const G1J* b) { const G1J x = *a, y = *b; *dst = g1_add_inl(x, y); }
 __device__ __noinline__ void g1_dbl_to(G1J* dst, const G1J* a) { const G1J x = *a; *dst = g1_dbl_inl(x); }
 
+__device__ __forceinline__ void msm_window_narrow(const G1JSlot* __restrict__ bucket_pts, const uint32_t* __restrict__ counts, G1JSlot* __restrict__ window_sums, const MsmPlan& p,
+                                                  uint32_t q, uint32_t k, G1J* lds) {
+    const uint32_t cls = p.narrow_q[q].cls;
+    if (!cls) return;
+    const MsmNarrowClass* nc = p.narrow + (cls - 1);
+    const uint32_t TN = nc->lanes, s = (k * blockDim.x + threadIdx.x) / TN, t = threadIdx.x % TN;
+    if (k * blockDim.x / TN >= nc->subs) return;
+    const bool live = s < nc->subs;
+    const uint32_t buckets = live ? 1u << (nc->sub[live ? s : 0].width - 1) : 0u, slice = buckets > TN ? buckets / TN : 1u;
+    const uint32_t lo = min(buckets, t * slice), hi = min(buckets, lo + slice);
+    G1J* run = lds + threadIdx.x;
+    G1J* sum = lds + blockDim.x + threadIdx.x;
+    G1J* scaled = lds + 2 * blockDim.x + threadIdx.x;
+    *run = G1J::identity(); *sum = G1J::identity();
+    const size_t bin0 = (size_t)q * p.windows * p.buckets + (live ? nc->sub[s].bin : 0u);
+    const G1JSlot* bp = bucket_pts + bin0;
+    const uint32_t* cn = counts + bin0;
+    for (uint32_t b = hi; b > lo; --b) {
+        if (cn[b - 1]) g1_add_to(run, run, &bp[b - 1].p);
+        g1_add_to(sum, sum, run);
+    }
+    if (lo < hi && t > 0) {
+        const int top = 31 - (int)__clz((int)t);
+        *scaled = *run;
+        for (int i = top - 1; i >= 0; --i) {
+            g1_dbl_to(scaled, scaled);
+            if ((t >> i) & 1) g1_add_to(scaled, scaled, run);
+        }
+        for (uint32_t w = slice; w > 1; w >>= 1) g1_dbl_to(scaled, scaled);
+        g1_add_to(sum, sum, scaled);
+    }
+    for (uint32_t d = TN / 2; d > 0; d >>= 1) {
+        const G1J mine_sum = *sum;
+        G1J other;
+        uint32_t* dst = reinterpret_cast<uint32_t*>(&other);
+        const uint32_t* src = reinterpret_cast<const uint32_t*>(&mine_sum);
+#pragma unroll
+        for (uint32_t j = 0; j < sizeof(G1J) / 4; ++j) dst[j] = (uint32_t)__shfl_down((int)src[j], d, 64);
+        if (t + d >= TN) other = G1J::identity();
+        *scaled = other;
+        g1_add_to(sum, sum, scaled);
+    }
+    if (t == 0 && live) window_sums[(size_t)p.narrow_q[q].sum_off + s] = *sum;
+}
+
 __global__ void __launch_bounds__(MSM_WIN_THREADS) msm_window(const G1JSlot* __restrict__ bucket_pts, const uint32_t* __restrict__ counts, G1JSlot* __restrict__ window_sums, MsmPlan p,
-                                                              uint32_t n_windows, uint32_t wpw, uint32_t slots) {
+                                                              uint32_t n_windows, uint32_t wpw, uint32_t slots, uint32_t wide_blocks, uint32_t narrow_blocks) {
     __builtin_amdgcn_s_setprio(3);
     extern __shared__ G1J win_lds[];
+    if (blockIdx.x >= wide_blocks) {
+        msm_window_narrow(bucket_pts, counts, window_sums, p, (blockIdx.x - wide_blocks) / narrow_blocks, (blockIdx.x - wide_blocks) % narrow_blocks, win_lds);
+        return;
+    }
     const uint32_t T = blockDim.x / wpw, sub = threadIdx.x / T, t = threadIdx.x % T;
     const uint32_t widx = blockIdx.x * wpw + sub;
-    const bool live = widx < n_windows;
+    bool live = widx < n_windows;
+    if (p.narrow) {
+        live = live && p.narrow_q[widx / p.windows].cls == 0;
+        if (!__syncthreads_or(live)) return;
+    }
     G1J* mine = win_lds + (size_t)sub * slots * T;
     G1J* run = mine + t;
     G1J* sum = mine + T + t;
@@ -789,7 +933,9 @@
     const uint32_t t = blockIdx.x * blockDim.x + threadIdx.x, q = t >> 2, r = t & 3u;
     if (q >= count) return;
     G1J acc = G1J::identity();
-    if (prs[q].n) acc = msm_horner_quad(window_sums + (size_t)q * p.windows, p.windows, p.c, r);
+    const uint32_t cls = p.narrow ? p.narrow_q[q].cls : 0u;
+    if (prs[q].n && cls) { const MsmNarrowClass* nc = p.narrow + (cls - 1); acc = msm_horner_quad_widths(window_sums + p.narrow_q[q].sum_off, nc->sub, nc->subs, r); }
+    else if (prs[q].n) acc = msm_horner_quad(window_sums + (size_t)q * p.windows, p.windows, p.c, r);
     if (r == 0) *prs[q].out = acc;
 }
 __global__ void __launch_bounds__(64) msm_final_parts(const G1JSlot* __restrict__ window_sums, const MsmProblem* __restrict__ prs, uint32_t count, MsmPlan p,
@@ -799,7 +945,12 @@
     if (quad >= count * parts) return;
     const uint32_t q = quad / parts, j = quad % parts, lo = j * wpp, hi = min(p.windows, lo + wpp);
     G1J acc = G1J::identity();
-    if (prs[q].n && lo < hi) acc = msm_horner_quad(window_sums + (size_t)q * p.windows + lo, hi - lo, p.c, r);
+    const uint32_t cls = p.narrow ? p.narrow_q[q].cls : 0u;
+    if (prs[q].n && cls) {
+        const MsmNarrowClass* nc = p.narrow + (cls - 1);
+        const uint32_t first = nc->piece_first[j], items = nc->piece_first[j + 1] - first;
+        if (items) acc = msm_horner_quad_widths(window_sums + p.narrow_q[q].sum_off + first, nc->sub + first, items, r);
+    } else if (prs[q].n && lo < hi) acc = msm_horner_quad(window_sums + (size_t)q * p.windows + lo, hi - lo, p.c, r);
     if (r == 0) out[quad] = acc;
     if (r == 0) { ready[quad].p.X = Fq::mul_inl(acc.X, acc.Z); ready[quad].p.Y = acc.Y; }
     if (r == 1) ready[quad].p.Z = Fq::mul_inl(acc.Z.sqr_inl(), acc.Z);
@@ -887,6 +1038,46 @@
     }
     return 0;
 }
+struct MsmNarrowLaunch { bool any = false; uint32_t problems = 0, classes = 0, max_subs = 0; size_t entries_nz = 0; MsmNarrowTable tab; std::vector<MsmNarrowProblem> q; };
+static void msm_narrow_plan(const MsmWorkspace& ws, const std::vector<MsmProblem>& v, const MsmPlan& p, uint32_t wpp, uint32_t nmax, MsmNarrowLaunch& N) {
+    memset(&N.tab, 0, sizeof(N.tab));
+    int class_of[32]; bool member[32] = {}, tried[32] = {};
+    for (int k = 0; k < 32; ++k) class_of[k] = -1;
+    auto key_of = [](uint32_t n) { int k = 0; while ((1u << k) < n) ++k; return k; };
+    for (const MsmProblem& q : v) if (q.n && q.n <= nmax / 2) member[key_of(q.n)] = true;
+    for (int k = 31; k >= 0; --k) {
+        if (!member[k] || N.classes == MSM_NARROW_CLASSES) continue;
+        tried[k] = true;
+        if (msm_narrow_class(p, wpp, nmax, 1u << k, N.tab.cls[N.classes])) class_of[k] = (int)N.classes++;
+        else memset(&N.tab.cls[N.classes], 0, sizeof(MsmNarrowClass));
+    }
+    if (!N.classes) return;
+    const uint32_t count = (uint32_t)v.size();
+    size_t dig = 0, sums = (size_t)count * p.windows;
+    for (const MsmProblem& q : v) {
+        int c = -1;
+        if (q.n && q.n <= nmax / 2) {
+            const int k = key_of(q.n);
+            c = class_of[k];
+            if (c < 0 && !tried[k]) for (int j = (int)N.classes - 1; j >= 0 && c < 0; --j) if (N.tab.cls[j].n_max >= q.n) c = j;
+        }
+        const uint32_t rows = c < 0 ? p.windows : N.tab.cls[c].subs;
+        N.q.push_back(MsmNarrowProblem{c < 0 ? 0u : (uint32_t)c + 1, (uint32_t)dig, c < 0 ? 0u : (uint32_t)sums});
+        dig += (size_t)rows * q.n;
+        if (c >= 0) { sums += rows; ++N.problems; N.max_subs = std::max(N.max_subs, rows); }
+        N.entries_nz += (size_t)(q.nnz ? std::min(q.nnz, q.n) : q.n) * 2 * rows;
+    }
+    N.any = N.problems > 0 && dig <= ws.glv.cap && sums <= ws.window_sums.cap && count <= ws.narrow_q.cap;
+    if (!N.any) { N.q.clear(); N.problems = 0; }
+}
+__global__ void msm_set_narrow_problems(MsmNarrowProblemChunk ch, uint32_t count, MsmNarrowProblem* __restrict__ dst) {
+    for (uint32_t i = threadIdx.x; i < count; i += blockDim.x) dst[i] = ch.q[i];
+}
+__global__ void msm_set_narrow(MsmNarrowTable tab, MsmNarrowClass* __restrict__ dst) {
+    const uint32_t* src = reinterpret_cast<const uint32_t*>(&tab);
+    uint32_t* d = reinterpret_cast<uint32_t*>(dst);
+    for (uint32_t i = threadIdx.x; i < sizeof(MsmNarrowTable) / 4; i += blockDim.x) d[i] = src[i];
+}
 static bool msm_same_problems(const std::vector<MsmProblem>& a, const std::vector<MsmProblem>& b) {
     if (a.size() != b.size()) return false;
     for (size_t i = 0; i < a.size(); ++i) {
@@ -905,28 +1096,70 @@
     const bool cut = L.cut;
     uint32_t nmax = L.nmax; const size_t total = L.total, total_nz = L.total_nz;
     const std::vector<MsmProblem>& launch_p = L.launch_p;
-    const bool uploaded = !ws.resident.empty() && ws.resident_no_split == ws.tune.msm_no_term_split && msm_same_problems(ws.resident, pr.p);
+    const uint32_t count = (uint32_t)L.launch_p.size();
+    MsmPlan p{0, 2, 0, 3};
+    uint32_t nbq = 0, nb = 0, stride = 0, piece_wpp = 0, piece_parts = 0, win_T = 0, win_wpw = 1, win_slots = MSM_WIN_SLOTS, narrow_blocks = 0;
+    size_t sort_lds = 0;
+    bool lds_sort = false;
+    MsmNarrowLaunch N;
+    if (nmax) {
+        if (nmax > MSM_ENTRY_TERM) { set_last_error("msm_enqueue_multi: more than 2^30 terms in one problem"); return H2V_ERR_BAD_ARGUMENT; }
+        if (total > ws.cap_terms) { set_last_error("msm_enqueue_multi: terms exceed workspace capacity"); return H2V_ERR_BAD_ARGUMENT; }
+        const bool latency = msm_latency_bound(total);
+        p = msm_plan(nmax, latency);
+        nbq = p.windows * p.buckets; nb = nbq * count;
+        if (nb > ws.cap_buckets || total * 2 * p.windows > ws.cap_list) { set_last_error("msm_enqueue_multi: workspace too small"); return H2V_ERR_BAD_ARGUMENT; }
+        stride = 2 * nmax;
+        sort_lds = ((size_t)p.buckets + MSM_SORT_THREADS) * 4 + (size_t)stride * 2;
+        lds_sort = nmax <= MSM_LDS_SORT_MAX_TERMS && sort_lds <= 150 * 1024 && (size_t)count * p.windows * stride <= ws.cap_list &&
+                   (size_t)count * p.windows <= (size_t)128 * ws.cap_problems && !ws.tune.msm_global_sort;
+        if (split && split->want_parts > 1 && p.windows > 1) {
+            const uint32_t want = std::min<uint32_t>(split->want_parts, MSM_MAX_PARTS);
+            piece_wpp = (p.windows + want - 1) / want; piece_parts = (p.windows + piece_wpp - 1) / piece_wpp;
+        }
+        if (lds_sort && !cut && !latency && count > 1) msm_narrow_plan(ws, L.launch_p, p, piece_wpp ? piece_wpp : p.windows, nmax, N);
+        {
+            const uint32_t nw = p.windows * count;
+            uint32_t T = msm_window_threads(p.buckets, nw, ws.tune.msm_window_threads), wpw = 1;
+            if (T == 64 && p.buckets >= 256 && nw > 256 && nw <= 512 && !ws.tune.msm_window_threads) { T = 128; wpw = 2; }
+            const uint32_t wpw_forced = (uint32_t)ws.tune.msm_window_wpw;
+            if ((wpw_forced == 1 || wpw_forced == 2 || wpw_forced == 4) && T * wpw_forced <= MSM_WIN_THREADS) wpw = wpw_forced;
+            win_slots = ((T * wpw <= 64 && nw > 1024) || ws.tune.msm_window_slots == 3) ? 3u : (uint32_t)MSM_WIN_SLOTS;
+            win_T = T; win_wpw = wpw;
+        }
+        if (N.any) {
+            const double wide_chain = msm_wide_chain(p.buckets, win_T, p.c);
+            for (uint32_t k = 0; k < N.classes; ++k) {
+                MsmNarrowClass& nc = N.tab.cls[k];
+                while (nc.lanes < 64 && nc.lanes < win_T * win_wpw && msm_narrow_chain(1u << (nc.c - 1), nc.lanes) > wide_chain) nc.lanes *= 2;
+                narrow_blocks = std::max(narrow_blocks, (nc.subs * nc.lanes + win_T * win_wpw - 1) / (win_T * win_wpw));
+            }
+        }
+    }
+    const bool uploaded = !ws.resident.empty() && ws.resident_no_split == ws.tune.msm_no_term_split && msm_same_problems(ws.resident, pr.p) &&
+                          ws.resident_narrow == N.any && (!N.any || memcmp(&N.tab, &ws.narrow_host, sizeof(MsmNarrowTable)) == 0);
     if (!uploaded) {
         if (cut) msm_upload_problems(s, L.parents_p, false, ws.parents.p);
         msm_upload_problems(s, launch_p, true, ws.problems.p);
-        ws.resident = pr.p; ws.resident_no_split = ws.tune.msm_no_term_split;
-    }
-    const uint32_t count = (uint32_t)launch_p.size();
+        if (N.any) {
+            hipLaunchKernelGGL(msm_set_narrow, dim3(1), dim3(256), 0, s, N.tab, ws.narrow_tab.p);
+            for (uint32_t q0 = 0; q0 < count; q0 += MSM_NARROW_PROBLEM_CHUNK) {
+                MsmNarrowProblemChunk ch;
+                const uint32_t k = std::min<uint32_t>(MSM_NARROW_PROBLEM_CHUNK, count - q0);
+                for (uint32_t i = 0; i < k; ++i) ch.q[i] = N.q[q0 + i];
+                hipLaunchKernelGGL(msm_set_narrow_problems, dim3(1), dim3(256), 0, s, ch, k, ws.narrow_q.p + q0);
+            }
+            ws.narrow_host = N.tab;
+        }
+        ws.resident = pr.p; ws.resident_no_split = ws.tune.msm_no_term_split; ws.resident_narrow = N.any;
+    }
+    if (N.any) { p.narrow = ws.narrow_tab.p; p.narrow_q = ws.narrow_q.p; }
     ws.final_problems = cut ? ws.parents.p : ws.problems.p;
     if (nmax == 0) {
         hipLaunchKernelGGL(msm_final, dim3((4 * count + 63) / 64), dim3(64), 0, s, ws.window_sums.p, ws.problems.p, count, MsmPlan{0, 2, 0, 3});
         H2V_HIP_CHECK(hipGetLastError());
         return 0;
     }
-    if (nmax > MSM_ENTRY_TERM) { set_last_error("msm_enqueue_multi: more than 2^30 terms in one problem"); return H2V_ERR_BAD_ARGUMENT; }
-    if (total > ws.cap_terms) { set_last_error("msm_enqueue_multi: terms exceed workspace capacity"); return H2V_ERR_BAD_ARGUMENT; }
-    MsmPlan p = msm_plan(nmax, msm_latency_bound(total));
-    uint32_t nbq = p.windows * p.buckets, nb = nbq * count;
-    if (nb > ws.cap_buckets || total * 2 * p.windows > ws.cap_list) { set_last_error("msm_enqueue_multi: workspace too small"); return H2V_ERR_BAD_ARGUMENT; }
-    const uint32_t stride = 2 * nmax;
-    const size_t sort_lds = ((size_t)p.buckets + MSM_SORT_THREADS) * 4 + (size_t)stride * 2;
-    const bool lds_sort = nmax <= MSM_LDS_SORT_MAX_TERMS && sort_lds <= 150 * 1024 && (size_t)count * p.windows * stride <= ws.cap_list &&
-                          (size_t)count * p.windows <= (size_t)128 * ws.cap_problems && !ws.tune.msm_global_sort;
     MsmSeg g;
     if (lds_sort) {
         hipLaunchKernelGGL(msm_glv_prep, dim3((nmax + 255) / 256, count), dim3(256), 0, s, ws.problems.p, count, p, ws.glv.p, ws.phi_pts.p);
@@ -949,7 +1182,7 @@
     hipLaunchKernelGGL(msm_count_or_scatter<true>, gt, dim3(MSM_TILE_THREADS), lds, s, ws.problems.p, count, tiles, p, wpp, ws.counts.p, ws.offsets.p, ws.cursor.p, ws.list.p);
     g = MsmSeg{ws.seg_start.p, 1, nb, 0, MSM_ACC_LANES_PER_ROUND};
     }
-    const uint32_t acc_blocks = msm_accumulate_blocks(total_nz * 2 * p.windows, MSM_ACC_LANES_PER_ROUND);
+    const uint32_t acc_blocks = msm_accumulate_blocks(N.any ? N.entries_nz : total_nz * 2 * p.windows, MSM_ACC_LANES_PER_ROUND);
     {
         const G1A* phi_tab = lds_sort ? (const G1A*)ws.phi_pts.p : (const G1A*)nullptr;
         if (ws.profile) {
@@ -960,24 +1193,19 @@
     hipLaunchKernelGGL(msm_accumulate_redo, dim3(256), dim3(64), 0, s, ws.problems.p, nbq, ws.counts.p, ws.offsets.p, ws.list.p, ws.bucket_pts.p, ws.partial.p, nb, g, ws.counts.p + nb, ws.cursor.p, ws.redo.p);
     hipLaunchKernelGGL(msm_fixup, dim3((nb + 63) / 64 + MSM_FIXUP_TEAM_BLOCKS + MSM_FIXUP_HEAVY_BLOCKS), dim3(64), 0, s, ws.counts.p, ws.offsets.p, ws.partial.p, ws.cursor.p, ws.bucket_pts.p, nb, g);
     {
-        const uint32_t nw = p.windows * count;
-        uint32_t T = msm_window_threads(p.buckets, nw, ws.tune.msm_window_threads), wpw = 1;
-        if (T == 64 && p.buckets >= 256 && nw > 256 && nw <= 512 && !ws.tune.msm_window_threads) { T = 128; wpw = 2; }
-        const uint32_t wpw_forced = (uint32_t)ws.tune.msm_window_wpw;
-        if ((wpw_forced == 1 || wpw_forced == 2 || wpw_forced == 4) && T * wpw_forced <= MSM_WIN_THREADS) wpw = wpw_forced;
-        const uint32_t slots = ((T * wpw <= 64 && nw > 1024) || ws.tune.msm_window_slots == 3) ? 3u : (uint32_t)MSM_WIN_SLOTS;
-        const size_t win_lds = (size_t)slots * T * wpw * sizeof(G1J);
+        const uint32_t nw = p.windows * count, wide_blocks = (nw + win_wpw - 1) / win_wpw;
+        const size_t win_lds = (size_t)win_slots * win_T * win_wpw * sizeof(G1J);
         if (win_lds > 64 * 1024) H2V_HIP_CHECK(hipFuncSetAttribute((const void*)msm_window, hipFuncAttributeMaxDynamicSharedMemorySize, (int)win_lds));
-        hipLaunchKernelGGL(msm_window, dim3((nw + wpw - 1) / wpw), dim3(T * wpw), win_lds, s, ws.bucket_pts.p, ws.counts.p, ws.window_sums.p, p, nw, wpw, slots);
+        hipLaunchKernelGGL(msm_window, dim3(wide_blocks + count * narrow_blocks), dim3(win_T * win_wpw), win_lds, s, ws.bucket_pts.p, ws.counts.p, ws.window_sums.p, p, nw, win_wpw, win_slots,
+                           wide_blocks, narrow_blocks);
     }
     const G1JSlot* sums = ws.window_sums.p;
     if (cut) {
         hipLaunchKernelGGL(msm_merge_windows, dim3((8 * n_callers * p.windows + 63) / 64), dim3(64), 0, s, ws.window_sums.p, ws.parents.p, n_callers, p.windows, ws.merged_sums.p);
         sums = ws.merged_sums.p;
     }
-    if (split && split->want_parts > 1 && p.windows > 1) {
-        const uint32_t want = std::min<uint32_t>(split->want_parts, MSM_MAX_PARTS);
-        const uint32_t wpp = (p.windows + want - 1) / want, parts = (p.windows + wpp - 1) / wpp;
+    if (piece_wpp) {
+        const uint32_t wpp = piece_wpp, parts = piece_parts;
         hipLaunchKernelGGL(msm_final_parts, dim3((4 * n_callers * parts + 63) / 64), dim3(64), 0, s, sums, ws.final_problems, n_callers, p, parts, wpp, ws.pieces.p, ws.pieces.p + (size_t)MSM_MAX_PARTS * ws.cap_problems);
         split->parts = parts; split->shift = p.c * wpp; split->count = n_callers; split->pts = ws.pieces.p; split->ready = ws.pieces.p + (size_t)MSM_MAX_PARTS * ws.cap_problems;
     } else {
```

New measurement: 11.30 million. 0.962x the previous value.
